# Yoii-Inc/zk-mpc

Hardware: AMD Instinct MI355X
Metric: R1CS constraints/sec (prove), Groth16 BLS12-377 (higher is better)
Workload: dtype u32x13 (29-bit limbs, int64 accumulate); 1 GPU; mul-chain R1CS, n=2^20-2 constraints, QAP domain 2^20, local prove; constraints=1048574, parties=1

## Files before the change

bindings/hip_ffi.rs:

```rust
#![allow(non_camel_case_types, dead_code, clippy::too_many_arguments)]
use std::os::raw::{c_char, c_void};

pub const ZK_OK: i32 = 0;
pub const ZK_ERR_HIP: i32 = -1;
pub const ZK_ERR_ARG: i32 = -2;
pub const ZK_ERR_NOMEM: i32 = -3;
pub const ZK_ERR_STATE: i32 = -4;
pub const ZK_ERR_MAC: i32 = -5;
pub const ZK_OP_MUL: i32 = 0;
pub const ZK_OP_ADD: i32 = 1;
pub const ZK_OP_SUB: i32 = 2;
pub const ZK_OP_NEG: i32 = 3;
pub const ZK_GT_EXPONENT_MULTIPLE: i32 = 3;

#[repr(C)] pub struct ZkCtx { _private: [u8; 0] }
#[repr(C)] pub struct ZkBases { _private: [u8; 0] }
#[repr(C)] pub struct ZkR1cs { _private: [u8; 0] }
#[repr(C)] pub struct ZkPk { _private: [u8; 0] }
#[repr(C)] pub struct ZkRng { _private: [u8; 0] }

#[repr(C)]
#[derive(Clone, Copy)]
pub struct ZkFr {
    pub l: [u64; 4],
// ... 199 lines not shown
    pub fn zk_fr_vec_op_dev(ctx: *mut ZkCtx, op: i32, a_dev: *const c_void, b_dev: *const c_void, out_dev: *mut c_void, n: usize) -> i32;
    pub fn zk_fr_vec_scale_dev(ctx: *mut ZkCtx, a_dev: *const c_void, k_host: *const ZkFr, out_dev: *mut c_void, n: usize) -> i32;
    pub fn zk_fr_batch_product_in_place(ctx: *mut ZkCtx, selfs_host: *mut ZkFr, others_host: *const ZkFr, n: usize) -> i32;
    pub fn zk_fr_ntt_dev(ctx: *mut ZkCtx, buf_dev: *mut c_void, log_n: u32, inverse: i32, coset: i32) -> i32;
    pub fn zk_fr_fft_in_place(ctx: *mut ZkCtx, vec_host: *mut ZkFr, n: usize, log_n: u32, inverse: i32, coset: i32) -> i32;
    pub fn zk_fr_divide_by_vanishing_on_coset_dev(ctx: *mut ZkCtx, evals_dev: *mut c_void, log_n: u32) -> i32;
    pub fn zk_fr_divide_by_vanishing_on_coset_in_place(ctx: *mut ZkCtx, evals_host: *mut ZkFr, log_n: u32) -> i32;
    pub fn zk_msm_g1(ctx: *mut ZkCtx, bases_host: *const ZkG1Affine, n_bases: usize, scalars_host: *const ZkFr, n_scalars: usize, out_host: *mut ZkG1Projective) -> i32;
    pub fn zk_msm_g2(ctx: *mut ZkCtx, bases_host: *const ZkG2Affine, n_bases: usize, scalars_host: *const ZkFr, n_scalars: usize, out_host: *mut ZkG2Projective) -> i32;
    pub fn zk_msm_g1_strided(ctx: *mut ZkCtx, bases_host: *const c_void, n_bases: usize, layout: *const ZkAffineLayout, scalars_host: *const ZkFr, n_scalars: usize, out_host: *mut ZkG1Projective) -> i32;
    pub fn zk_msm_g2_strided(ctx: *mut ZkCtx, bases_host: *const c_void, n_bases: usize, layout: *const ZkAffineLayout, scalars_host: *const ZkFr, n_scalars: usize, out_host: *mut ZkG2Projective) -> i32;
    pub fn zk_bases_cache_config(ctx: *mut ZkCtx, budget_bytes: usize, precompute_after: i32) -> i32;
    pub fn zk_bases_cache_trust(ctx: *mut ZkCtx, fingerprint_only: i32) -> i32;
    pub fn zk_bases_cache_drop(ctx: *mut ZkCtx) -> i32;
    pub fn zk_bases_cache_sync(ctx: *mut ZkCtx) -> i32;
    pub fn zk_bases_cache_stats(ctx: *mut ZkCtx, out: *mut u64 ) -> i32;
    pub fn zk_bases_cache_stats2(ctx: *mut ZkCtx, out: *mut u64 ) -> i32;
    pub fn zk_msm_speculate(ctx: *mut ZkCtx, on: i32) -> i32;
    pub fn zk_msm_speculate_stats(ctx: *mut ZkCtx, out: *mut u64 ) -> i32;
    pub fn zk_bases_upload_g1(ctx: *mut ZkCtx, bases_host: *const ZkG1Affine, n: usize, out: *mut *mut ZkBases) -> i32;
    pub fn zk_bases_upload_g2(ctx: *mut ZkCtx, bases_host: *const ZkG2Affine, n: usize, out: *mut *mut ZkBases) -> i32;
    pub fn zk_bases_free(ctx: *mut ZkCtx, b: *mut ZkBases) -> i32;
    pub fn zk_bases_precompute(ctx: *mut ZkCtx, b: *mut ZkBases) -> i32;
    pub fn zk_bases_precompute_as(ctx: *mut ZkCtx, b: *mut ZkBases, layout: i32) -> i32;
    pub fn zk_bases_precompute_note(b: *const ZkBases) -> *const c_char;
    pub fn zk_bases_window_bits(b: *const ZkBases) -> u32;
    pub fn zk_bases_len(b: *const ZkBases) -> usize;
    pub fn zk_msm_g1_dev(ctx: *mut ZkCtx, bases: *const ZkBases, base_offset: usize, scalars_dev: *const c_void, n: usize, out_host: *mut ZkG1Projective) -> i32;
    pub fn zk_msm_g2_dev(ctx: *mut ZkCtx, bases: *const ZkBases, base_offset: usize, scalars_dev: *const c_void, n: usize, out_host: *mut ZkG2Projective) -> i32;
    pub fn zk_msm_g1_multi_dev(ctx: *mut ZkCtx, bases: *const ZkBases, base_offset: usize, scalars_dev: *const c_void, n: usize, stride: usize, count: usize, outs_host: *mut ZkG1Projective) -> i32;
    pub fn zk_msm_g2_multi_dev(ctx: *mut ZkCtx, bases: *const ZkBases, base_offset: usize, scalars_dev: *const c_void, n: usize, stride: usize, count: usize, outs_host: *mut ZkG2Projective) -> i32;
    pub fn zk_fixed_base_g1_dev(ctx: *mut ZkCtx, gen_k_host: *const ZkFr, scalars_dev: *const c_void, n: usize, out: *mut *mut ZkBases) -> i32;
    pub fn zk_fixed_base_g2_dev(ctx: *mut ZkCtx, gen_k_host: *const ZkFr, scalars_dev: *const c_void, n: usize, out: *mut *mut ZkBases) -> i32;
    pub fn zk_bases_download_g1(ctx: *mut ZkCtx, b: *const ZkBases, offset: usize, n: usize, out_host: *mut ZkG1Affine) -> i32;
    pub fn zk_bases_download_g2(ctx: *mut ZkCtx, b: *const ZkBases, offset: usize, n: usize, out_host: *mut ZkG2Affine) -> i32;
    pub fn zk_point_serialized_size(group: i32, compressed: i32) -> usize;
    pub fn zk_bases_serialize(ctx: *mut ZkCtx, b: *const ZkBases, offset: usize, n: usize, compressed: i32, out_host: *mut u8) -> i32;
    pub fn zk_bases_deserialize_uncompressed(ctx: *mut ZkCtx, group: i32, bytes_host: *const u8, n: usize, out: *mut *mut ZkBases) -> i32;
    pub fn zk_bases_deserialize_compressed(ctx: *mut ZkCtx, group: i32, bytes_host: *const u8, n: usize, out: *mut *mut ZkBases) -> i32;
    pub fn zk_vk_serialized_size(pk: *const ZkPk, compressed: i32) -> usize;
    pub fn zk_pk_serialized_size(pk: *const ZkPk, compressed: i32) -> usize;
    pub fn zk_vk_serialize(ctx: *mut ZkCtx, pk: *const ZkPk, compressed: i32, out_host: *mut u8, cap: usize) -> i32;
    pub fn zk_pk_serialize(ctx: *mut ZkCtx, pk: *const ZkPk, compressed: i32, out_host: *mut u8, cap: usize) -> i32;
    pub fn zk_pk_deserialize(ctx: *mut ZkCtx, bytes_host: *const u8, len: usize, compressed: i32, out: *mut *mut ZkPk) -> i32;
    pub fn zk_kzg_srs_serialized_size(n_powers_g: usize, n_powers_gamma_g: usize, compressed: i32) -> usize;
    pub fn zk_kzg_srs_serialize(ctx: *mut ZkCtx, powers_g: *const ZkBases, powers_gamma_g: *const ZkBases, h: *const ZkG2Affine, beta_h: *const ZkG2Affine, compressed: i32, out_host: *mut u8, cap: usize) -> i32;
    pub fn zk_kzg_srs_deserialize(ctx: *mut ZkCtx, bytes_host: *const u8, len: usize, compressed: i32, powers_g: *mut *mut ZkBases, powers_gamma_g: *mut *mut ZkBases, h: *mut ZkG2Affine, beta_h: *mut ZkG2Affine) -> i32;
    pub fn zk_msm_batch_dev(ctx: *mut ZkCtx, n_jobs: usize, bases: *const *const ZkBases, base_offsets: *const usize, scalars_dev: *const *const c_void, lens: *const usize, outs: *const *mut c_void) -> i32;
    pub fn zk_g1_add(a: *const ZkG1Projective, b: *const ZkG1Projective, out: *mut ZkG1Projective) -> i32;
    pub fn zk_g2_add(a: *const ZkG2Projective, b: *const ZkG2Projective, out: *mut ZkG2Projective) -> i32;
    pub fn zk_g1_neg(a: *const ZkG1Projective, out: *mut ZkG1Projective) -> i32;
    pub fn zk_g2_neg(a: *const ZkG2Projective, out: *mut ZkG2Projective) -> i32;
    pub fn zk_g1_mul(a: *const ZkG1Projective, k: *const ZkFr, out: *mut ZkG1Projective) -> i32;
    pub fn zk_g2_mul(a: *const ZkG2Projective, k: *const ZkFr, out: *mut ZkG2Projective) -> i32;
    pub fn zk_g1_from_affine(a: *const ZkG1Affine, out: *mut ZkG1Projective) -> i32;
    pub fn zk_g2_from_affine(a: *const ZkG2Affine, out: *mut ZkG2Projective) -> i32;
    pub fn zk_g1_serialize(a: *const ZkG1Projective, out: *mut u8 ) -> i32;
    pub fn zk_g2_serialize(a: *const ZkG2Projective, out: *mut u8 ) -> i32;
    pub fn zk_fr_add(a: *const ZkFr, b: *const ZkFr, out: *mut ZkFr) -> i32;
    pub fn zk_fr_sub(a: *const ZkFr, b: *const ZkFr, out: *mut ZkFr) -> i32;
    pub fn zk_fr_mul(a: *const ZkFr, b: *const ZkFr, out: *mut ZkFr) -> i32;
    pub fn zk_fq_add(a: *const ZkFq, b: *const ZkFq, out: *mut ZkFq) -> i32;
    pub fn zk_fq_sub(a: *const ZkFq, b: *const ZkFq, out: *mut ZkFq) -> i32;
    pub fn zk_fq_mul(a: *const ZkFq, b: *const ZkFq, out: *mut ZkFq) -> i32;
    pub fn zk_fq_neg5_almost_raw(a13: *const u32 , out13: *mut u32 ) -> i32;
    pub fn zk_fr_lazy_raw(op: i32, in9s: *const u32, out9s: *mut u32) -> i32;
    pub fn zk_fq_lazy_raw(op: i32, in13s: *const u32, out13s: *mut u32) -> i32;
    pub fn zk_fq_mul2(a: *const ZkFq, b: *const ZkFq, c: *const ZkFq, d: *const ZkFq, out: *mut ZkFq) -> i32;
    pub fn zk_fr_inverse(a: *const ZkFr, out: *mut ZkFr) -> i32;
    pub fn zk_fr_pow(a: *const ZkFr, e: u64, out: *mut ZkFr) -> i32;
    pub fn zk_fr_from_canonical(canon: *const u64 , out: *mut ZkFr) -> i32;
    pub fn zk_fr_to_canonical(a: *const ZkFr, canon: *mut u64 ) -> i32;
    pub fn zk_r1cs_upload(ctx: *mut ZkCtx, m: *const ZkR1csHost, out: *mut *mut ZkR1cs) -> i32;
    pub fn zk_r1cs_free(ctx: *mut ZkCtx, r: *mut ZkR1cs) -> i32;
    pub fn zk_r1cs_mul_chain(ctx: *mut ZkCtx, n: usize, out: *mut *mut ZkR1cs) -> i32;
    pub fn zk_mul_chain_assignment_dev(ctx: *mut ZkCtx, n: usize, w0: *const ZkFr, w1: *const ZkFr, z_dev: *mut c_void) -> i32;
    pub fn zk_pk_upload(ctx: *mut ZkCtx, pk: *const ZkPkHost, out: *mut *mut ZkPk) -> i32;
    pub fn zk_pk_free(ctx: *mut ZkCtx, pk: *mut ZkPk) -> i32;
    pub fn zk_groth16_setup(ctx: *mut ZkCtx, r1cs: *const ZkR1cs, alpha: *const ZkFr, beta: *const ZkFr, gamma: *const ZkFr, delta: *const ZkFr, tau: *const ZkFr, g1_k: *const ZkFr, g2_k: *const ZkFr, out: *mut *mut ZkPk) -> i32;
    pub fn zk_pk_query_len(pk: *const ZkPk, which: i32) -> usize;
    pub fn zk_pk_query_bases(pk: *const ZkPk, which: i32) -> *const ZkBases;
    pub fn zk_msm_mul_levels(ctx: *mut ZkCtx, levels: i32) -> i32;
    pub fn zk_pk_mul_levels(pk: *const ZkPk) -> u32;
    pub fn zk_msm_mul_levels_clamp(window_bits: u32, levels: u32) -> u32;
    pub fn zk_pk_download_g1(ctx: *mut ZkCtx, pk: *const ZkPk, which: i32, offset: usize, n: usize, out: *mut ZkG1Affine) -> i32;
    pub fn zk_pk_download_g2(ctx: *mut ZkCtx, pk: *const ZkPk, which: i32, offset: usize, n: usize, out: *mut ZkG2Affine) -> i32;
    pub fn zk_pk_vk_g1(pk: *const ZkPk, which: i32, out: *mut ZkG1Affine) -> i32;
    pub fn zk_pk_vk_g2(pk: *const ZkPk, which: i32, out: *mut ZkG2Affine) -> i32;
    pub fn zk_groth16_witness_map_dev(ctx: *mut ZkCtx, r1cs: *const ZkR1cs, z_dev: *const c_void, h_dev: *mut c_void) -> i32;
    pub fn zk_r1cs_domain_log(r1cs: *const ZkR1cs) -> u32;
    pub fn zk_groth16_witness_map_pre_dev(ctx: *mut ZkCtx, r1cs: *const ZkR1cs, z_dev: *const c_void, include_instance: i32, a_dev: *mut c_void, b_dev: *mut c_void, c_dev: *mut c_void) -> i32;
    pub fn zk_groth16_witness_map_post_dev(ctx: *mut ZkCtx, r1cs: *const ZkR1cs, ab_dev: *mut c_void, c_dev: *const c_void) -> i32;
    pub fn zk_groth16_hint_next_dev(ctx: *mut ZkCtx, z_next_dev: *const c_void) -> i32;
    pub fn zk_groth16_chain_fronts(ctx: *mut ZkCtx, on: i32) -> i32;
    pub fn zk_groth16_msms_presort_dev(ctx: *mut ZkCtx, pk: *const ZkPk, r1cs: *const ZkR1cs, z_dev: *const c_void) -> i32;
    pub fn zk_groth16_msms_begin_dev(ctx: *mut ZkCtx, pk: *const ZkPk, r: *const ZkR1cs, z: *const c_void) -> i32;
    pub fn zk_groth16_msms_dev(ctx: *mut ZkCtx, pk: *const ZkPk, r1cs: *const ZkR1cs, z_dev: *const c_void, h_dev: *const c_void, out_g1: *mut ZkG1Projective , out_g2: *mut ZkG2Projective) -> i32;
    pub fn zk_groth16_prove_dev(ctx: *mut ZkCtx, pk: *const ZkPk, r1cs: *const ZkR1cs, z_dev: *const c_void, r: *const ZkFr, s: *const ZkFr, proof_out: *mut u8 ) -> i32;
    pub fn zk_groth16_prove_batch_dev(ctx: *mut ZkCtx, pk: *const ZkPk, r1cs: *const ZkR1cs, count: usize, z_dev: *const c_void, r: *const ZkFr, s: *const ZkFr, proofs_out: *mut u8) -> i32;
    pub fn zk_groth16_prove_batch(ctx: *mut ZkCtx, pk: *const ZkPk, r1cs: *const ZkR1cs, count: usize, z_host: *const ZkFr, r: *const ZkFr, s: *const ZkFr, proofs_out: *mut u8) -> i32;
    pub fn zk_groth16_prove_multi(ctxs: *const *mut ZkCtx, pks: *const *const ZkPk, r1css: *const *const ZkR1cs, n_ctx: i32, z_dev0: *const c_void, r: *const ZkFr, s: *const ZkFr, proof_out: *mut u8 ) -> i32;
    pub fn zk_groth16_multi_plan(pk: *const ZkPk, r1cs: *const ZkR1cs, n_ctx: i32, out: *mut c_char, cap: usize, written: *mut usize) -> i32;
    pub fn zk_groth16_prove(ctx: *mut ZkCtx, pk: *const ZkPk, r1cs: *const ZkR1cs, z_host: *const ZkFr, r: *const ZkFr, s: *const ZkFr, proof_out: *mut u8 ) -> i32;
    pub fn zk_groth16_prove_queued(ctx: *mut ZkCtx, pk: *const ZkPk, r1cs: *const ZkR1cs, z_host: *const ZkFr, r: *const ZkFr, s: *const ZkFr, z_next_host: *const ZkFr, proof_out: *mut u8 ) -> i32;
    pub fn zk_gt_exponent_multiple() -> i32;
    pub fn zk_pairing_products(ctx: *mut ZkCtx, p: *const ZkG1Affine, q: *const ZkG2Affine, pairs: usize, count: usize, outs: *mut ZkGt) -> i32;
    pub fn zk_pairing_products_host(p: *const ZkG1Affine, q: *const ZkG2Affine, pairs: usize, count: usize, outs: *mut ZkGt) -> i32;
    pub fn zk_gt_is_one(a: *const ZkGt) -> i32;
    pub fn zk_gt_eq(a: *const ZkGt, b: *const ZkGt) -> i32;
    pub fn zk_gt_mul(a: *const ZkGt, b: *const ZkGt, out: *mut ZkGt) -> i32;
    pub fn zk_groth16_verify_batch(ctx: *mut ZkCtx, pk: *const ZkPk, count: usize, inputs_host: *const ZkFr, inputs_per_proof: usize, proofs_host: *const u8, ok: *mut i32) -> i32;
    pub fn zk_groth16_verify_host(vk: *const ZkVkHost, inputs: *const ZkFr, n_inputs: usize, proof: *const u8 , ok: *mut i32) -> i32;
    pub fn zk_marlin_verify_host(vk: *const ZkMarlinVkHost, inputs: *const ZkFr, n_inputs: usize, proof: *const u8, proof_len: usize, ok: *mut i32) -> i32;
    pub fn zk_marlin_verify_batch(ctx: *mut ZkCtx, vk: *const ZkMarlinVkHost, count: usize, inputs_host: *const ZkFr, inputs_per_proof: usize, proofs_host: *const u8, offsets: *const usize, ok: *mut i32) -> i32;
    pub fn zk_fr_powers_dev(ctx: *mut ZkCtx, base: *const ZkFr, start: *const ZkFr, n: usize, out_dev: *mut c_void) -> i32;
    pub fn zk_fr_batch_inverse_dev(ctx: *mut ZkCtx, v_dev: *mut c_void, n: usize) -> i32;
    pub fn zk_poly_evaluate_dev(ctx: *mut ZkCtx, coeffs_dev: *const c_void, n: usize, point: *const ZkFr, out: *mut ZkFr) -> i32;
    pub fn zk_poly_evaluate_batch_dev(ctx: *mut ZkCtx, polys: *const ZkPolyRef, points: *const ZkFr, count: usize, out: *mut ZkFr) -> i32;
    pub fn zk_poly_divide_by_linear_dev(ctx: *mut ZkCtx, coeffs_dev: *const c_void, n: usize, z: *const ZkFr, q_dev: *mut c_void, rem: *mut ZkFr) -> i32;
    pub fn zk_poly_divide_by_vanishing_dev(ctx: *mut ZkCtx, coeffs_dev: *const c_void, n: usize, log_domain: u32, q_dev: *mut c_void, r_dev: *mut c_void) -> i32;
    pub fn zk_poly_mul_dev(ctx: *mut ZkCtx, a_dev: *const c_void, na: usize, b_dev: *const c_void, nb: usize, out_dev: *mut c_void) -> i32;
    pub fn zk_kzg_commit_dev(ctx: *mut ZkCtx, powers_g: *const ZkBases, coeffs_dev: *const c_void, n: usize, powers_gamma_g: *const ZkBases, blind_dev: *const c_void, n_blind: usize, out: *mut ZkG1Projective) -> i32;
    pub fn zk_kzg_open_dev(ctx: *mut ZkCtx, powers_g: *const ZkBases, coeffs_dev: *const c_void, n: usize, point: *const ZkFr, powers_gamma_g: *const ZkBases, blind_dev: *const c_void, n_blind: usize, w_out: *mut ZkG1Projective, random_v_out: *mut ZkFr) -> i32;
    pub fn zk_r1cs_matvec_dev(ctx: *mut ZkCtx, r1cs: *const ZkR1cs, which: i32, z_dev: *const c_void, out_dev: *mut c_void, out_len: usize) -> i32;
    pub fn zk_fr_gather_dev(ctx: *mut ZkCtx, src_dev: *const c_void, idx_dev: *const u32, n: usize, out_dev: *mut c_void) -> i32;
    pub fn zk_marlin_round3_f_evals_dev(ctx: *mut ZkCtx, on_k: *const ZkMarlinMatrixEvals , k_size: usize, alpha: *const ZkFr, beta: *const ZkFr, eta: *const ZkFr , vh_alpha_vh_beta: *const ZkFr, f_out_dev: *mut c_void) -> i32;
    pub fn zk_marlin_round3_ab_evals_dev(ctx: *mut ZkCtx, on_b: *const ZkMarlinMatrixEvals , b_size: usize, alpha: *const ZkFr, beta: *const ZkFr, eta: *const ZkFr , vh_alpha_vh_beta: *const ZkFr, a_out_dev: *mut c_void, b_out_dev: *mut c_void) -> i32;
    pub fn zk_marlin_proof_max_size() -> usize;
    pub fn zk_marlin_prove(ctx: *mut ZkCtx, index: *const ZkMarlinIndex, powers_g: *const ZkBases, powers_gamma_g: *const ZkBases, z_dev: *const c_void, zk_rng: *mut ZkRng, mask_on_device: i32, proof_out: *mut u8, cap: usize, proof_len: *mut usize) -> i32;
    pub fn zk_she_vec_op_dev(ctx: *mut ZkCtx, op: i32, a_dev: *const c_void, b_dev: *const c_void, out_dev: *mut c_void, n: usize) -> i32;
    pub fn zk_she_vec_scale_dev(ctx: *mut ZkCtx, a_dev: *const c_void, k: *const ZkFq753, out_dev: *mut c_void, n: usize) -> i32;
    pub fn zk_she_negacyclic_mul_dev(ctx: *mut ZkCtx, a_dev: *const c_void, b_dev: *const c_void, out_dev: *mut c_void, n: usize, batch: usize) -> i32;
    pub fn zk_she_ciphertext_mul_dev(ctx: *mut ZkCtx, x_dev: *const c_void, y_dev: *const c_void, out_dev: *mut c_void, n: usize, batch: usize) -> i32;
    pub fn zk_she_encrypt_dev(ctx: *mut ZkCtx, e_dev: *const c_void, pk_a_dev: *const c_void, pk_b_dev: *const c_void, r_dev: *const c_void, p: *const ZkFq753, out_dev: *mut c_void, n: usize, batch: usize) -> i32;
    pub fn zk_she_decrypt_dev(ctx: *mut ZkCtx, ct_dev: *const c_void, sk_dev: *const c_void, out_dev: *mut c_void, n: usize, batch: usize) -> i32;
    pub fn zk_she_encode_dev(ctx: *mut ZkCtx, plain_fr_dev: *const c_void, out_dev: *mut c_void, n: usize, batch: usize) -> i32;
    pub fn zk_she_decode_dev(ctx: *mut ZkCtx, enc_dev: *const c_void, out_fr_dev: *mut c_void, n: usize, batch: usize) -> i32;
    pub fn zk_comm_unique_id(out: *mut u8 ) -> i32;
    pub fn zk_comm_init(ctx: *mut ZkCtx, id: *const u8 , rank: i32, n_parties: i32) -> i32;
    pub fn zk_comm_destroy(ctx: *mut ZkCtx) -> i32;
    pub fn zk_comm_info(ctx: *mut ZkCtx, n_ranks: *mut i32, rank: *mut i32, device: *mut i32, rccl_version: *mut i32, lib_path: *mut c_char, lib_path_cap: usize) -> i32;
    pub fn zk_comm_set_open_pattern(ctx: *mut ZkCtx, pattern: i32) -> i32;
    pub fn zk_open_sum_fr_dev(ctx: *mut ZkCtx, v_dev: *const c_void, n: usize, out_dev: *mut c_void) -> i32;
    pub fn zk_groth16_prove_shared(ctx: *mut ZkCtx, pk: *const ZkPk, r1cs: *const ZkR1cs, z_share_dev: *const c_void, r_share: *const ZkFr, s_share: *const ZkFr, tx_dev: *const c_void, ty_dev: *const c_void, tz_dev: *const c_void, net: *const ZkNetVtable, proof: *mut u8 , bytes_sent: *mut u64) -> i32;
    pub fn zk_groth16_prove_shared_spdz(ctx: *mut ZkCtx, pk: *const ZkPk, r1cs: *const ZkR1cs, z_lanes_dev: *const *const c_void , r_lanes: *const ZkFr , s_lanes: *const ZkFr , tx_lanes_dev: *const *const c_void , ty_lanes_dev: *const *const c_void , tz_lanes_dev: *const *const c_void , net: *const ZkNetVtable, proof: *mut u8 , bytes_sent: *mut u64) -> i32;
    pub fn zk_marlin_prove_shared(ctx: *mut ZkCtx, index: *const ZkMarlinIndex, powers_g: *const ZkBases, powers_gamma_g: *const ZkBases, z_share_dev: *const c_void, zk_rng: *mut ZkRng, mask_on_device: i32, tx: *const c_void, ty: *const c_void, tz: *const c_void, net: *const ZkNetVtable, proof_out: *mut u8, cap: usize, proof_len: *mut usize, bytes_sent: *mut u64) -> i32;
    pub fn zk_marlin_prove_shared_spdz(ctx: *mut ZkCtx, index: *const ZkMarlinIndex, powers_g: *const ZkBases, powers_gamma_g: *const ZkBases, z_lanes_dev: *const *const c_void , zk_rng: *mut ZkRng, mask_on_device: i32, tx_lanes: *const *const c_void , ty_lanes: *const *const c_void , tz_lanes: *const *const c_void , net: *const ZkNetVtable, proof_out: *mut u8, cap: usize, proof_len: *mut usize, bytes_sent: *mut u64) -> i32;
    pub fn zk_mpc_fft_in_place(ctx: *mut ZkCtx, vec_host: *mut c_void, n: usize, layout: *const ZkMpcFieldLayout, log_n: u32, inverse: i32, coset: i32) -> i32;
    pub fn zk_mpc_divide_by_vanishing_on_coset_in_place(ctx: *mut ZkCtx, evals_host: *mut c_void, layout: *const ZkMpcFieldLayout, log_n: u32) -> i32;
    pub fn zk_mpc_batch_product_in_place(ctx: *mut ZkCtx, selfs_host: *mut c_void, others_host: *const c_void, n: usize, layout: *const ZkMpcFieldLayout, triple_host: *const *const ZkFr, net: *const ZkNetVtable, bytes_sent: *mut u64) -> i32;
    pub fn zk_mpc_msm_g1(ctx: *mut ZkCtx, bases_host: *const c_void, n_bases: usize, base_layout: *const ZkMpcGroupLayout, scalars_host: *const c_void, n_scalars: usize, scalar_layout: *const ZkMpcFieldLayout, out_lanes: *mut ZkG1Projective , scalars_public: *mut i32) -> i32;
    pub fn zk_mpc_msm_g2(ctx: *mut ZkCtx, bases_host: *const c_void, n_bases: usize, base_layout: *const ZkMpcGroupLayout, scalars_host: *const c_void, n_scalars: usize, scalar_layout: *const ZkMpcFieldLayout, out_lanes: *mut ZkG2Projective , scalars_public: *mut i32) -> i32;
    pub fn zk_fr_sum_parties_dev(ctx: *mut ZkCtx, gathered_dev: *const c_void, n_parties: usize, n: usize, out_dev: *mut c_void) -> i32;
    pub fn zk_beaver_combine_dev(ctx: *mut ZkCtx, sx_open_dev: *const c_void, oy_open_dev: *const c_void, tx_dev: *const c_void, ty_dev: *const c_void, tz_dev: *const c_void, out_dev: *mut c_void, n: usize) -> i32;
    pub fn zk_fr_vec_is_zero_dev(ctx: *mut ZkCtx, v_dev: *const c_void, n: usize, is_zero: *mut i32) -> i32;
    pub fn zk_fr_random_dev(ctx: *mut ZkCtx, key32: *const u8, stream_id: u64, out_dev: *mut c_void, n: usize) -> i32;
    pub fn zk_fsrng_new(seed_bytes: *const u8, len: usize, out: *mut *mut ZkRng) -> i32;
    pub fn zk_fsrng_absorb(rng: *mut ZkRng, bytes: *const u8, len: usize) -> i32;
    pub fn zk_rng_from_seed(seed: *const u8 , rounds: i32, out: *mut *mut ZkRng) -> i32;
    pub fn zk_rng_free(rng: *mut ZkRng) -> i32;
    pub fn zk_rng_next_u64(rng: *mut ZkRng, out: *mut u64) -> i32;
    pub fn zk_rng_next_u128(rng: *mut ZkRng, out: *mut u64 ) -> i32;
    pub fn zk_rng_next_fr(rng: *mut ZkRng, out: *mut ZkFr) -> i32;
    pub fn zk_rng_fill_fr(rng: *mut ZkRng, out: *mut ZkFr, n: usize) -> i32;
    pub fn zk_rng_fill_bytes(rng: *mut ZkRng, out: *mut u8, n: usize) -> i32;
    pub fn zk_blake2s(data: *const u8, len: usize, out: *mut u8 ) -> i32;
// ... 17 lines not shown
```

include/zkmpc_hip.h:

```cpp
#ifndef ZKMPC_HIP_H
#define ZKMPC_HIP_H

#include <stddef.h>
#include <stdint.h>

#ifdef __cplusplus
extern "C" {
#endif

#define ZK_OK 0
#define ZK_ERR_HIP -1
#define ZK_ERR_ARG -2
#define ZK_ERR_NOMEM -3
#define ZK_ERR_STATE -4
#define ZK_ERR_MAC -5

typedef struct zk_ctx zk_ctx;
typedef struct zk_bases zk_bases;
typedef struct zk_r1cs zk_r1cs;
typedef struct zk_pk zk_pk;
typedef struct zk_rng zk_rng;

typedef struct { uint64_t l[4]; } zk_fr;
typedef struct { uint64_t l[6]; } zk_fq;
// ... 63 lines not shown
                  size_t n, zk_g2_projective* out_host);
int zk_msm_g1_multi_dev(zk_ctx* ctx, const zk_bases* bases, size_t base_offset, const void* scalars_dev,
                        size_t n, size_t stride, size_t count, zk_g1_projective* outs_host);
int zk_msm_g2_multi_dev(zk_ctx* ctx, const zk_bases* bases, size_t base_offset, const void* scalars_dev,
                        size_t n, size_t stride, size_t count, zk_g2_projective* outs_host);
int zk_fixed_base_g1_dev(zk_ctx* ctx, const zk_fr* gen_k_host, const void* scalars_dev, size_t n, zk_bases** out);
int zk_fixed_base_g2_dev(zk_ctx* ctx, const zk_fr* gen_k_host, const void* scalars_dev, size_t n, zk_bases** out);
int zk_bases_download_g1(zk_ctx* ctx, const zk_bases* b, size_t offset, size_t n, zk_g1_affine* out_host);
int zk_bases_download_g2(zk_ctx* ctx, const zk_bases* b, size_t offset, size_t n, zk_g2_affine* out_host);

size_t zk_point_serialized_size(int group, int compressed);
int zk_bases_serialize(zk_ctx* ctx, const zk_bases* b, size_t offset, size_t n, int compressed, uint8_t* out_host);
int zk_bases_deserialize_uncompressed(zk_ctx* ctx, int group, const uint8_t* bytes_host, size_t n, zk_bases** out);
int zk_bases_deserialize_compressed(zk_ctx* ctx, int group, const uint8_t* bytes_host, size_t n, zk_bases** out);

size_t zk_vk_serialized_size(const zk_pk* pk, int compressed);
size_t zk_pk_serialized_size(const zk_pk* pk, int compressed);
int zk_vk_serialize(zk_ctx* ctx, const zk_pk* pk, int compressed, uint8_t* out_host, size_t cap);
int zk_pk_serialize(zk_ctx* ctx, const zk_pk* pk, int compressed, uint8_t* out_host, size_t cap);
int zk_pk_deserialize(zk_ctx* ctx, const uint8_t* bytes_host, size_t len, int compressed, zk_pk** out);
size_t zk_kzg_srs_serialized_size(size_t n_powers_g, size_t n_powers_gamma_g, int compressed);
int zk_kzg_srs_serialize(zk_ctx* ctx, const zk_bases* powers_g, const zk_bases* powers_gamma_g, const zk_g2_affine* h,
                         const zk_g2_affine* beta_h, int compressed, uint8_t* out_host, size_t cap);
int zk_kzg_srs_deserialize(zk_ctx* ctx, const uint8_t* bytes_host, size_t len, int compressed, zk_bases** powers_g,
                           zk_bases** powers_gamma_g, zk_g2_affine* h, zk_g2_affine* beta_h);

int zk_msm_batch_dev(zk_ctx* ctx, size_t n_jobs, const zk_bases* const* bases, const size_t* base_offsets,
                     const void* const* scalars_dev, const size_t* lens, void* const* outs);

int zk_g1_add(const zk_g1_projective* a, const zk_g1_projective* b, zk_g1_projective* out);
int zk_g2_add(const zk_g2_projective* a, const zk_g2_projective* b, zk_g2_projective* out);
int zk_g1_neg(const zk_g1_projective* a, zk_g1_projective* out);
int zk_g2_neg(const zk_g2_projective* a, zk_g2_projective* out);
int zk_g1_mul(const zk_g1_projective* a, const zk_fr* k, zk_g1_projective* out);
int zk_g2_mul(const zk_g2_projective* a, const zk_fr* k, zk_g2_projective* out);
int zk_g1_from_affine(const zk_g1_affine* a, zk_g1_projective* out);
int zk_g2_from_affine(const zk_g2_affine* a, zk_g2_projective* out);
int zk_g1_serialize(const zk_g1_projective* a, uint8_t out[48]);
int zk_g2_serialize(const zk_g2_projective* a, uint8_t out[96]);
int zk_fr_add(const zk_fr* a, const zk_fr* b, zk_fr* out);
int zk_fr_sub(const zk_fr* a, const zk_fr* b, zk_fr* out);
int zk_fr_mul(const zk_fr* a, const zk_fr* b, zk_fr* out);
int zk_fq_add(const zk_fq* a, const zk_fq* b, zk_fq* out);
int zk_fq_sub(const zk_fq* a, const zk_fq* b, zk_fq* out);
int zk_fq_mul(const zk_fq* a, const zk_fq* b, zk_fq* out);
int zk_fq_neg5_almost_raw(const uint32_t a13[13], uint32_t out13[13]);
int zk_fr_lazy_raw(int op, const uint32_t* in9s, uint32_t* out9s);
int zk_fq_lazy_raw(int op, const uint32_t* in13s, uint32_t* out13s);
int zk_fq_mul2(const zk_fq* a, const zk_fq* b, const zk_fq* c, const zk_fq* d, zk_fq* out);
int zk_fr_inverse(const zk_fr* a, zk_fr* out);
int zk_fr_pow(const zk_fr* a, uint64_t e, zk_fr* out);
int zk_fr_from_canonical(const uint64_t canon[4], zk_fr* out);
int zk_fr_to_canonical(const zk_fr* a, uint64_t canon[4]);

typedef struct {
    size_t num_constraints, num_instance, num_witness;
    const uint32_t* a_row_ptr; const uint32_t* a_col; const zk_fr* a_coeff;
    const uint32_t* b_row_ptr; const uint32_t* b_col; const zk_fr* b_coeff;
    const uint32_t* c_row_ptr; const uint32_t* c_col; const zk_fr* c_coeff;
} zk_r1cs_host;
int zk_r1cs_upload(zk_ctx* ctx, const zk_r1cs_host* m, zk_r1cs** out);
int zk_r1cs_free(zk_ctx* ctx, zk_r1cs* r);
int zk_r1cs_mul_chain(zk_ctx* ctx, size_t n, zk_r1cs** out);
int zk_mul_chain_assignment_dev(zk_ctx* ctx, size_t n, const zk_fr* w0, const zk_fr* w1, void* z_dev);

typedef struct {
    zk_g1_affine alpha_g1, beta_g1, delta_g1;
    zk_g2_affine beta_g2, delta_g2;
    const zk_g1_affine* a_query;    size_t a_len;
    const zk_g1_affine* b_g1_query; size_t b_g1_len;
    const zk_g2_affine* b_g2_query; size_t b_g2_len;
    const zk_g1_affine* h_query;    size_t h_len;
    const zk_g1_affine* l_query;    size_t l_len;
} zk_pk_host;
int zk_pk_upload(zk_ctx* ctx, const zk_pk_host* pk, zk_pk** out);
int zk_pk_free(zk_ctx* ctx, zk_pk* pk);
int zk_groth16_setup(zk_ctx* ctx, const zk_r1cs* r1cs, const zk_fr* alpha, const zk_fr* beta,
                     const zk_fr* gamma, const zk_fr* delta, const zk_fr* tau,
                     const zk_fr* g1_k, const zk_fr* g2_k, zk_pk** out);
size_t zk_pk_query_len(const zk_pk* pk, int which);
const zk_bases* zk_pk_query_bases(const zk_pk* pk, int which);
int zk_msm_mul_levels(zk_ctx* ctx, int levels);
uint32_t zk_pk_mul_levels(const zk_pk* pk);
uint32_t zk_msm_mul_levels_clamp(uint32_t window_bits, uint32_t levels);
int zk_pk_download_g1(zk_ctx* ctx, const zk_pk* pk, int which, size_t offset, size_t n, zk_g1_affine* out);
int zk_pk_download_g2(zk_ctx* ctx, const zk_pk* pk, int which, size_t offset, size_t n, zk_g2_affine* out);
int zk_pk_vk_g1(const zk_pk* pk, int which, zk_g1_affine* out);
int zk_pk_vk_g2(const zk_pk* pk, int which, zk_g2_affine* out);

int zk_groth16_witness_map_dev(zk_ctx* ctx, const zk_r1cs* r1cs, const void* z_dev, void* h_dev);
uint32_t zk_r1cs_domain_log(const zk_r1cs* r1cs);
int zk_groth16_witness_map_pre_dev(zk_ctx* ctx, const zk_r1cs* r1cs, const void* z_dev,
                                   int include_instance, void* a_dev, void* b_dev, void* c_dev);
int zk_groth16_witness_map_post_dev(zk_ctx* ctx, const zk_r1cs* r1cs, void* ab_dev, const void* c_dev);
int zk_groth16_hint_next_dev(zk_ctx* ctx, const void* z_next_dev);
int zk_groth16_chain_fronts(zk_ctx* ctx, int on);
int zk_groth16_msms_presort_dev(zk_ctx* ctx, const zk_pk* pk, const zk_r1cs* r1cs, const void* z_dev);
int zk_groth16_msms_begin_dev(zk_ctx* ctx, const zk_pk* pk, const zk_r1cs* r, const void* z);
int zk_groth16_msms_dev(zk_ctx* ctx, const zk_pk* pk, const zk_r1cs* r1cs, const void* z_dev,
                        const void* h_dev, zk_g1_projective out_g1[4], zk_g2_projective* out_g2);
int zk_groth16_prove_dev(zk_ctx* ctx, const zk_pk* pk, const zk_r1cs* r1cs, const void* z_dev,
                         const zk_fr* r, const zk_fr* s, uint8_t proof_out[192]);
int zk_groth16_prove_batch_dev(zk_ctx* ctx, const zk_pk* pk, const zk_r1cs* r1cs, size_t count, const void* z_dev,
                               const zk_fr* r, const zk_fr* s, uint8_t* proofs_out);
int zk_groth16_prove_batch(zk_ctx* ctx, const zk_pk* pk, const zk_r1cs* r1cs, size_t count, const zk_fr* z_host,
                           const zk_fr* r, const zk_fr* s, uint8_t* proofs_out);
int zk_groth16_prove_multi(zk_ctx* const* ctxs, const zk_pk* const* pks, const zk_r1cs* const* r1css, int n_ctx, const void* z_dev0,
                           const zk_fr* r, const zk_fr* s, uint8_t proof_out[192]);
int zk_groth16_multi_plan(const zk_pk* pk, const zk_r1cs* r1cs, int n_ctx, char* out, size_t cap, size_t* written);
int zk_groth16_prove(zk_ctx* ctx, const zk_pk* pk, const zk_r1cs* r1cs, const zk_fr* z_host,
                     const zk_fr* r, const zk_fr* s, uint8_t proof_out[192]);
int zk_groth16_prove_queued(zk_ctx* ctx, const zk_pk* pk, const zk_r1cs* r1cs, const zk_fr* z_host,
                            const zk_fr* r, const zk_fr* s, const zk_fr* z_next_host, uint8_t proof_out[192]);

#define ZK_GT_EXPONENT_MULTIPLE 3
int zk_gt_exponent_multiple(void);
typedef struct { zk_fq c[12]; } zk_gt;
int zk_pairing_products(zk_ctx* ctx, const zk_g1_affine* p, const zk_g2_affine* q, size_t pairs, size_t count, zk_gt* outs);
int zk_pairing_products_host(const zk_g1_affine* p, const zk_g2_affine* q, size_t pairs, size_t count, zk_gt* outs);
int zk_gt_is_one(const zk_gt* a);
int zk_gt_eq(const zk_gt* a, const zk_gt* b);
int zk_gt_mul(const zk_gt* a, const zk_gt* b, zk_gt* out);
int zk_groth16_verify_batch(zk_ctx* ctx, const zk_pk* pk, size_t count, const zk_fr* inputs_host, size_t inputs_per_proof,
                            const uint8_t* proofs_host, int* ok);
typedef struct {
    zk_g1_affine alpha_g1;
    zk_g2_affine beta_g2, gamma_g2, delta_g2;
    const zk_g1_affine* gamma_abc_g1; size_t gamma_abc_len;
} zk_vk_host;
int zk_groth16_verify_host(const zk_vk_host* vk, const zk_fr* inputs, size_t n_inputs, const uint8_t proof[192], int* ok);

typedef struct {
    const uint8_t* ivk_bytes; size_t ivk_len;
    zk_g1_affine g, gamma_g;
    zk_g2_affine h, beta_h;
    zk_g1_affine shift_h, shift_k;
} zk_marlin_vk_host;
int zk_marlin_verify_host(const zk_marlin_vk_host* vk, const zk_fr* inputs, size_t n_inputs, const uint8_t* proof, size_t proof_len, int* ok);
int zk_marlin_verify_batch(zk_ctx* ctx, const zk_marlin_vk_host* vk, size_t count, const zk_fr* inputs_host, size_t inputs_per_proof,
                           const uint8_t* proofs_host, const size_t* offsets, int* ok);

int zk_fr_powers_dev(zk_ctx* ctx, const zk_fr* base, const zk_fr* start, size_t n, void* out_dev);
int zk_fr_batch_inverse_dev(zk_ctx* ctx, void* v_dev, size_t n);
int zk_poly_evaluate_dev(zk_ctx* ctx, const void* coeffs_dev, size_t n, const zk_fr* point, zk_fr* out);
typedef struct { const void* ptr; size_t n; } zk_poly_ref;
int zk_poly_evaluate_batch_dev(zk_ctx* ctx, const zk_poly_ref* polys, const zk_fr* points, size_t count, zk_fr* out);
int zk_poly_divide_by_linear_dev(zk_ctx* ctx, const void* coeffs_dev, size_t n, const zk_fr* z, void* q_dev, zk_fr* rem);
int zk_poly_divide_by_vanishing_dev(zk_ctx* ctx, const void* coeffs_dev, size_t n, uint32_t log_domain, void* q_dev, void* r_dev);
int zk_poly_mul_dev(zk_ctx* ctx, const void* a_dev, size_t na, const void* b_dev, size_t nb, void* out_dev);
int zk_kzg_commit_dev(zk_ctx* ctx, const zk_bases* powers_g, const void* coeffs_dev, size_t n,
                      const zk_bases* powers_gamma_g, const void* blind_dev, size_t n_blind, zk_g1_projective* out);
int zk_kzg_open_dev(zk_ctx* ctx, const zk_bases* powers_g, const void* coeffs_dev, size_t n, const zk_fr* point,
                    const zk_bases* powers_gamma_g, const void* blind_dev, size_t n_blind,
                    zk_g1_projective* w_out, zk_fr* random_v_out);

int zk_r1cs_matvec_dev(zk_ctx* ctx, const zk_r1cs* r1cs, int which, const void* z_dev, void* out_dev, size_t out_len);
int zk_fr_gather_dev(zk_ctx* ctx, const void* src_dev, const uint32_t* idx_dev, size_t n, void* out_dev);
typedef struct { const void* row; const void* col; const void* val; const void* row_col; } zk_marlin_matrix_evals;
int zk_marlin_round3_f_evals_dev(zk_ctx* ctx, const zk_marlin_matrix_evals on_k[3], size_t k_size, const zk_fr* alpha,
                                 const zk_fr* beta, const zk_fr eta[3], const zk_fr* vh_alpha_vh_beta, void* f_out_dev);
int zk_marlin_round3_ab_evals_dev(zk_ctx* ctx, const zk_marlin_matrix_evals on_b[3], size_t b_size, const zk_fr* alpha,
                                  const zk_fr* beta, const zk_fr eta[3], const zk_fr* vh_alpha_vh_beta, void* a_out_dev,
                                  void* b_out_dev);

typedef struct {
    size_t num_constraints, num_variables, num_non_zero, num_instance;
// ... 112 lines not shown
```

zk-mpc_amd/_lib.py:

```python
from __future__ import annotations

import ctypes as C
import os

_HERE = os.path.dirname(os.path.abspath(__file__))
LIB_PATH = os.path.join(_HERE, "lib", "libzkmpc_hip.so")

ZK_OK = 0
OP_MUL, OP_ADD, OP_SUB, OP_NEG = 0, 1, 2, 3


class ZkError(RuntimeError):
    pass


class Fr(C.Structure):
    _fields_ = [("l", C.c_uint64 * 4)]


class Fq(C.Structure):
    _fields_ = [("l", C.c_uint64 * 6)]


class MarlinMatrixEvals(C.Structure):
# ... 74 lines not shown
    "zk_ctx_sync": (_I, [_P]),
    "zk_ctx_stream": (_P, [_P]),
    "zk_version": (_I, []),
    "zk_groth16_prove_shared": (_I, [_P, _P, _P, _P, _P, _P, _P, _P, _P, _P, _P, _P]),
    "zk_groth16_prove_shared_spdz": (_I, [_P, _P, _P, _P, _P, _P, _P, _P, _P, _P, _P, _P]),
    "zk_selftest_exception_barrier": (_I, [_I]),
    "zk_dev_alloc": (_I, [_P, _SZ, C.POINTER(_P)]),
    "zk_dev_free": (_I, [_P, _P]),
    "zk_memcpy_h2d": (_I, [_P, _P, _P, _SZ]),
    "zk_memcpy_d2h": (_I, [_P, _P, _P, _SZ]),
    "zk_fr_vec_op_dev": (_I, [_P, _I, _P, _P, _P, _SZ]),
    "zk_fr_vec_scale_dev": (_I, [_P, _P, _P, _P, _SZ]),
    "zk_fr_batch_product_in_place": (_I, [_P, _P, _P, _SZ]),
    "zk_fr_ntt_dev": (_I, [_P, _P, _U32, _I, _I]),
    "zk_fr_fft_in_place": (_I, [_P, _P, _SZ, _U32, _I, _I]),
    "zk_fr_divide_by_vanishing_on_coset_dev": (_I, [_P, _P, _U32]),
    "zk_msm_g1": (_I, [_P, _P, _SZ, _P, _SZ, _P]),
    "zk_msm_g2": (_I, [_P, _P, _SZ, _P, _SZ, _P]),
    "zk_msm_g1_strided": (_I, [_P, _P, _SZ, _P, _P, _SZ, _P]),
    "zk_msm_g2_strided": (_I, [_P, _P, _SZ, _P, _P, _SZ, _P]),
    "zk_bases_cache_config": (_I, [_P, _SZ, _I]),
    "zk_bases_cache_trust": (_I, [_P, _I]),
    "zk_msm_speculate": (_I, [_P, _I]),
    "zk_msm_speculate_stats": (_I, [_P, _P]),
    "zk_bases_cache_drop": (_I, [_P]),
    "zk_bases_cache_sync": (_I, [_P]),
    "zk_bases_cache_stats": (_I, [_P, _P]),
    "zk_bases_cache_stats2": (_I, [_P, _P]),
    "zk_mpc_fft_in_place": (_I, [_P, _P, _SZ, _P, _U32, _I, _I]),
    "zk_mpc_divide_by_vanishing_on_coset_in_place": (_I, [_P, _P, _P, _U32]),
    "zk_mpc_batch_product_in_place": (_I, [_P, _P, _P, _SZ, _P, _P, _P, _P]),
    "zk_mpc_msm_g1": (_I, [_P, _P, _SZ, _P, _P, _SZ, _P, _P, _P]),
    "zk_mpc_msm_g2": (_I, [_P, _P, _SZ, _P, _P, _SZ, _P, _P, _P]),
    "zk_fr_divide_by_vanishing_on_coset_in_place": (_I, [_P, _P, _U32]),
    "zk_bases_upload_g1": (_I, [_P, _P, _SZ, C.POINTER(_P)]),
    "zk_bases_upload_g2": (_I, [_P, _P, _SZ, C.POINTER(_P)]),
    "zk_bases_free": (_I, [_P, _P]),
    "zk_bases_precompute": (_I, [_P, _P]),
    "zk_bases_precompute_as": (_I, [_P, _P, _I]),
    "zk_bases_precompute_note": (C.c_char_p, [_P]),
    "zk_bases_len": (_SZ, [_P]),
    "zk_bases_window_bits": (_U32, [_P]),
    "zk_msm_g1_dev": (_I, [_P, _P, _SZ, _P, _SZ, _P]),
    "zk_msm_g2_dev": (_I, [_P, _P, _SZ, _P, _SZ, _P]),
    "zk_msm_g1_multi_dev": (_I, [_P, _P, _SZ, _P, _SZ, _SZ, _SZ, _P]),
    "zk_msm_g2_multi_dev": (_I, [_P, _P, _SZ, _P, _SZ, _SZ, _SZ, _P]),
    "zk_fixed_base_g1_dev": (_I, [_P, _P, _P, _SZ, C.POINTER(_P)]),
    "zk_fixed_base_g2_dev": (_I, [_P, _P, _P, _SZ, C.POINTER(_P)]),
    "zk_bases_download_g1": (_I, [_P, _P, _SZ, _SZ, _P]),
    "zk_bases_download_g2": (_I, [_P, _P, _SZ, _SZ, _P]),
    "zk_g1_add": (_I, [_P, _P, _P]),
    "zk_g2_add": (_I, [_P, _P, _P]),
    "zk_g1_neg": (_I, [_P, _P]),
    "zk_g2_neg": (_I, [_P, _P]),
    "zk_g1_mul": (_I, [_P, _P, _P]),
    "zk_g2_mul": (_I, [_P, _P, _P]),
    "zk_g1_from_affine": (_I, [_P, _P]),
    "zk_g2_from_affine": (_I, [_P, _P]),
    "zk_g1_serialize": (_I, [_P, _P]),
    "zk_g2_serialize": (_I, [_P, _P]),
    "zk_fr_add": (_I, [_P, _P, _P]),
    "zk_fr_sub": (_I, [_P, _P, _P]),
    "zk_fr_mul": (_I, [_P, _P, _P]),
    "zk_fq_add": (_I, [_P, _P, _P]),
    "zk_fq_sub": (_I, [_P, _P, _P]),
    "zk_fq_mul": (_I, [_P, _P, _P]),
    "zk_fq_mul2": (_I, [_P, _P, _P, _P, _P]),
    "zk_fq_neg5_almost_raw": (_I, [_P, _P]),
    "zk_fq_lazy_raw": (_I, [_I, _P, _P]),
    "zk_fr_lazy_raw": (_I, [_I, _P, _P]),
    "zk_fr_from_canonical": (_I, [_P, _P]),
    "zk_fr_to_canonical": (_I, [_P, _P]),
    "zk_r1cs_upload": (_I, [_P, _P, C.POINTER(_P)]),
    "zk_r1cs_free": (_I, [_P, _P]),
    "zk_r1cs_mul_chain": (_I, [_P, _SZ, C.POINTER(_P)]),
    "zk_mul_chain_assignment_dev": (_I, [_P, _SZ, _P, _P, _P]),
    "zk_pk_upload": (_I, [_P, _P, C.POINTER(_P)]),
    "zk_pk_free": (_I, [_P, _P]),
    "zk_groth16_setup": (_I, [_P, _P, _P, _P, _P, _P, _P, _P, _P, C.POINTER(_P)]),
    "zk_pk_query_len": (_SZ, [_P, _I]),
    "zk_pk_query_bases": (_P, [_P, _I]),
    "zk_msm_mul_levels": (_I, [_P, _I]),
    "zk_pk_mul_levels": (_U32, [_P]),
    "zk_msm_mul_levels_clamp": (_U32, [_U32, _U32]),
    "zk_pk_download_g1": (_I, [_P, _P, _I, _SZ, _SZ, _P]),
    "zk_pk_download_g2": (_I, [_P, _P, _I, _SZ, _SZ, _P]),
    "zk_pk_vk_g1": (_I, [_P, _I, _P]),
    "zk_pk_vk_g2": (_I, [_P, _I, _P]),
    "zk_groth16_witness_map_dev": (_I, [_P, _P, _P, _P]),
    "zk_r1cs_domain_log": (_U32, [_P]),
    "zk_groth16_witness_map_pre_dev": (_I, [_P, _P, _P, _I, _P, _P, _P]),
    "zk_groth16_witness_map_post_dev": (_I, [_P, _P, _P, _P]),
    "zk_groth16_msms_dev": (_I, [_P, _P, _P, _P, _P, _P, _P]),
    "zk_groth16_msms_presort_dev": (_I, [_P, _P, _P, _P]),
    "zk_groth16_msms_begin_dev": (_I, [_P, _P, _P, _P]),
    "zk_groth16_hint_next_dev": (_I, [_P, _P]),
    "zk_groth16_chain_fronts": (_I, [_P, _I]),
    "zk_groth16_prove_dev": (_I, [_P, _P, _P, _P, _P, _P, _P]),
    "zk_groth16_prove_batch_dev": (_I, [_P, _P, _P, _SZ, _P, _P, _P, _P]),
    "zk_groth16_prove_batch": (_I, [_P, _P, _P, _SZ, _P, _P, _P, _P]),
    "zk_groth16_prove_multi": (_I, [_P, _P, _P, _I, _P, _P, _P, _P]),
    "zk_groth16_multi_plan": (_I, [_P, _P, _I, C.c_char_p, _SZ, C.POINTER(_SZ)]),
    "zk_groth16_prove": (_I, [_P, _P, _P, _P, _P, _P, _P]),
    "zk_groth16_prove_queued": (_I, [_P, _P, _P, _P, _P, _P, _P, _P]),
    "zk_host_alloc": (_I, [_P, _SZ, C.POINTER(_P)]),
    "zk_host_free": (_I, [_P, _P]),
    "zk_fr_powers_dev": (_I, [_P, _P, _P, _SZ, _P]),
    "zk_fr_batch_inverse_dev": (_I, [_P, _P, _SZ]),
    "zk_poly_evaluate_dev": (_I, [_P, _P, _SZ, _P, _P]),
    "zk_poly_evaluate_batch_dev": (_I, [_P, _P, _P, _SZ, _P]),
    "zk_poly_divide_by_linear_dev": (_I, [_P, _P, _SZ, _P, _P, _P]),
    "zk_poly_divide_by_vanishing_dev": (_I, [_P, _P, _SZ, _U32, _P, _P]),
    "zk_poly_mul_dev": (_I, [_P, _P, _SZ, _P, _SZ, _P]),
    "zk_kzg_commit_dev": (_I, [_P, _P, _P, _SZ, _P, _P, _SZ, _P]),
    "zk_kzg_open_dev": (_I, [_P, _P, _P, _SZ, _P, _P, _P, _SZ, _P, _P]),
    "zk_point_serialized_size": (_SZ, [_I, _I]),
    "zk_bases_serialize": (_I, [_P, _P, _SZ, _SZ, _I, _P]),
    "zk_bases_deserialize_uncompressed": (_I, [_P, _I, _P, _SZ, C.POINTER(_P)]),
    "zk_bases_deserialize_compressed": (_I, [_P, _I, _P, _SZ, C.POINTER(_P)]),
    "zk_msm_batch_dev": (_I, [_P, _SZ, _P, _P, _P, _P, _P]),
    "zk_vk_serialized_size": (_SZ, [_P, _I]),
    "zk_pk_serialized_size": (_SZ, [_P, _I]),
    "zk_vk_serialize": (_I, [_P, _P, _I, _P, _SZ]),
    "zk_pk_serialize": (_I, [_P, _P, _I, _P, _SZ]),
    "zk_pk_deserialize": (_I, [_P, _P, _SZ, _I, C.POINTER(_P)]),
    "zk_kzg_srs_serialized_size": (_SZ, [_SZ, _SZ, _I]),
    "zk_kzg_srs_serialize": (_I, [_P, _P, _P, _P, _P, _I, _P, _SZ]),
    "zk_kzg_srs_deserialize": (_I, [_P, _P, _SZ, _I, C.POINTER(_P), C.POINTER(_P), _P, _P]),
    "zk_comm_unique_id": (_I, [_P]),
    "zk_comm_init": (_I, [_P, _P, _I, _I]),
    "zk_comm_destroy": (_I, [_P]),
    "zk_comm_info": (_I, [_P, C.POINTER(_I), C.POINTER(_I), C.POINTER(_I), C.POINTER(_I), C.c_char_p, _SZ]),
    "zk_comm_set_open_pattern": (_I, [_P, _I]),
    "zk_open_sum_fr_dev": (_I, [_P, _P, _SZ, _P]),
    "zk_memcpy_d2d": (_I, [_P, _P, _P, _SZ]),
    "zk_dev_zero": (_I, [_P, _P, _SZ]),
    "zk_fr_inverse": (_I, [_P, _P]),
    "zk_fr_pow": (_I, [_P, C.c_uint64, _P]),
    "zk_r1cs_matvec_dev": (_I, [_P, _P, _I, _P, _P, _SZ]),
    "zk_fr_gather_dev": (_I, [_P, _P, _P, _SZ, _P]),
    "zk_marlin_round3_f_evals_dev": (_I, [_P, _P, _SZ, _P, _P, _P, _P, _P]),
    "zk_marlin_round3_ab_evals_dev": (_I, [_P, _P, _SZ, _P, _P, _P, _P, _P, _P]),
    "zk_marlin_proof_max_size": (_SZ, []),
    "zk_marlin_prove": (_I, [_P, _P, _P, _P, _P, _P, _I, _P, _SZ, _P]),
    "zk_marlin_prove_shared": (_I, [_P, _P, _P, _P, _P, _P, _I, _P, _P, _P, _P, _P, _SZ, _P, _P]),
    "zk_marlin_prove_shared_spdz": (_I, [_P, _P, _P, _P, _P, _P, _I, _P, _P, _P, _P, _P, _SZ, _P, _P]),
    "zk_she_vec_op_dev": (_I, [_P, _I, _P, _P, _P, _SZ]),
    "zk_she_vec_scale_dev": (_I, [_P, _P, _P, _P, _SZ]),
    "zk_she_negacyclic_mul_dev": (_I, [_P, _P, _P, _P, _SZ, _SZ]),
    "zk_she_ciphertext_mul_dev": (_I, [_P, _P, _P, _P, _SZ, _SZ]),
    "zk_she_encrypt_dev": (_I, [_P, _P, _P, _P, _P, _P, _P, _SZ, _SZ]),
    "zk_she_decrypt_dev": (_I, [_P, _P, _P, _P, _SZ, _SZ]),
    "zk_she_encode_dev": (_I, [_P, _P, _P, _SZ, _SZ]),
    "zk_she_decode_dev": (_I, [_P, _P, _P, _SZ, _SZ]),
    "zk_fr_sum_parties_dev": (_I, [_P, _P, _SZ, _SZ, _P]),
    "zk_beaver_combine_dev": (_I, [_P, _P, _P, _P, _P, _P, _P, _SZ]),
    "zk_fr_vec_is_zero_dev": (_I, [_P, _P, _SZ, _P]),
    "zk_fr_random_dev": (_I, [_P, _P, C.c_uint64, _P, _SZ]),
    "zk_fsrng_new": (_I, [_P, _SZ, C.POINTER(_P)]),
    "zk_fsrng_absorb": (_I, [_P, _P, _SZ]),
    "zk_rng_from_seed": (_I, [_P, _I, C.POINTER(_P)]),
    "zk_rng_free": (_I, [_P]),
    "zk_rng_next_u64": (_I, [_P, _P]),
    "zk_rng_next_u128": (_I, [_P, _P]),
    "zk_rng_next_fr": (_I, [_P, _P]),
    "zk_rng_fill_fr": (_I, [_P, _P, _SZ]),
# ... 47 lines not shown
```

zk-mpc_amd/api.py:

```python
from __future__ import annotations

import ctypes as C

import numpy as np

from . import _lib
from ._lib import ZkError


def _ptr(a: np.ndarray):
    return a.ctypes.data_as(C.c_void_p)


def _fr_struct(limbs4) -> _lib.Fr:
    f = _lib.Fr()
    for i in range(4):
        f.l[i] = int(limbs4[i])
    return f


class HostBuf:

    def __init__(self, ctx: "Context", nbytes: int):
        self.ctx, self.nbytes = ctx, nbytes
# ... 768 lines not shown
        return out

    def groth16_verify_batch(self, pk: "ProvingKey", inputs_mont: np.ndarray, proofs) -> np.ndarray:
        data = b"".join(proofs) if isinstance(proofs, (list, tuple)) else bytes(proofs)
        if len(data) % 192:
            raise ValueError("proofs must be a whole number of 192-byte proofs")
        count = len(data) // 192
        inp = np.ascontiguousarray(inputs_mont, dtype=np.uint64).reshape(count, -1, 4) if count else np.zeros((0, 0, 4), np.uint64)
        buf = np.frombuffer(data, dtype=np.uint8)
        ok = np.zeros(count, dtype=np.int32)
        self._ck(self.lib.zk_groth16_verify_batch(self.h, pk.h, count, _ptr(inp), inp.shape[1], _ptr(buf), _ptr(ok)))
        return ok

    def groth16_verify(self, pk: "ProvingKey", inputs_mont: np.ndarray, proof: bytes) -> bool:
        return bool(self.groth16_verify_batch(pk, np.asarray(inputs_mont, dtype=np.uint64).reshape(1, -1, 4), proof)[0])

    def diag_fq12(self, op: int, a: np.ndarray, b: np.ndarray) -> np.ndarray:
        cases = np.ascontiguousarray(np.stack([a, b], axis=1), dtype=np.uint64)
        out = np.zeros((cases.shape[0], 72), dtype=np.uint64)
        self._ck(self.lib.zk_diag_fq12_dev(self.h, op, _ptr(cases), _ptr(out), cases.shape[0]))
        return out


class Bases:
    def __init__(self, ctx: Context, h, group: int, owned: bool = True):
        self.ctx, self.h, self.group, self.owned = ctx, h, group, owned

    def __len__(self):
        return self.ctx.lib.zk_bases_len(self.h)

    def precompute(self, layout: int = 0):
        if layout:
            self.ctx._ck(self.ctx.lib.zk_bases_precompute_as(self.ctx.h, self.h, layout))
        else:
            self.ctx._ck(self.ctx.lib.zk_bases_precompute(self.ctx.h, self.h))

    def precompute_note(self) -> str:
        return (self.ctx.lib.zk_bases_precompute_note(self.h) or b"").decode()

    def download(self, offset: int = 0, n: int = None) -> np.ndarray:
        n = len(self) - offset if n is None else n
        out = np.zeros((n, 12 if self.group == 1 else 24), dtype=np.uint64)
        fn = self.ctx.lib.zk_bases_download_g1 if self.group == 1 else self.ctx.lib.zk_bases_download_g2
        self.ctx._ck(fn(self.ctx.h, self.h, offset, n, _ptr(out)))
        return out

    def serialize(self, compressed: bool = True, offset: int = 0, n: int = None) -> bytes:
        n = len(self) - offset if n is None else n
        per = self.ctx.lib.zk_point_serialized_size(self.group, int(compressed))
        out = np.zeros(max(n * per, 1), dtype=np.uint8)
        self.ctx._ck(self.ctx.lib.zk_bases_serialize(self.ctx.h, self.h, offset, n, int(compressed), _ptr(out)))
        return out[: n * per].tobytes()

    def free(self):
        if self.h and self.owned:
            self.ctx.lib.zk_bases_free(self.ctx.h, self.h)
        self.h = None


class R1cs:
    def __init__(self, ctx: Context, h, nc: int, ni: int, nw: int):
        self.ctx, self.h = ctx, h
        self.num_constraints, self.num_instance, self.num_witness = nc, ni, nw

    @property
    def domain_log(self) -> int:
        return self.ctx.lib.zk_r1cs_domain_log(self.h)

    def free(self):
        if self.h:
            self.ctx.lib.zk_r1cs_free(self.ctx.h, self.h)
            self.h = None


class ProvingKey:
    QUERIES = {"a_query": 0, "b_g1_query": 1, "b_g2_query": 2, "h_query": 3, "l_query": 4, "gamma_abc_g1": 5}

    def __init__(self, ctx: Context, h):
        self.ctx, self.h = ctx, h

    def mul_levels(self) -> int:
        return self.ctx.lib.zk_pk_mul_levels(self.h)

    def query_len(self, name: str) -> int:
        return self.ctx.lib.zk_pk_query_len(self.h, self.QUERIES[name])

    def download(self, name: str, offset: int = 0, n: int = None) -> np.ndarray:
        which = self.QUERIES[name]
        n = self.query_len(name) - offset if n is None else n
        if which == 2:
            out = np.zeros((n, 24), dtype=np.uint64)
            self.ctx._ck(self.ctx.lib.zk_pk_download_g2(self.ctx.h, self.h, which, offset, n, _ptr(out)))
        else:
            out = np.zeros((n, 12), dtype=np.uint64)
            self.ctx._ck(self.ctx.lib.zk_pk_download_g1(self.ctx.h, self.h, which, offset, n, _ptr(out)))
        return out

    def query_bases(self, name: str) -> "Bases":
        which = self.QUERIES[name]
        h = self.ctx.lib.zk_pk_query_bases(self.h, which)
        return Bases(self.ctx, C.c_void_p(h), 2 if which == 2 else 1, owned=False)

    def vk_g1(self, which: int) -> np.ndarray:
        out = np.zeros(12, dtype=np.uint64)
        self.ctx._ck(self.ctx.lib.zk_pk_vk_g1(self.h, which, _ptr(out)))
        return out

    def vk_g2(self, which: int) -> np.ndarray:
        out = np.zeros(24, dtype=np.uint64)
        self.ctx._ck(self.ctx.lib.zk_pk_vk_g2(self.h, which, _ptr(out)))
        return out

    def verify_host(self, inputs_mont, proof: bytes) -> bool:
        return groth16_verify_host(self.vk_g1(0), self.vk_g2(0), self.vk_g2(2), self.vk_g2(1), self.download("gamma_abc_g1"), inputs_mont, proof)

    def free(self):
        if self.h:
            self.ctx.lib.zk_pk_free(self.ctx.h, self.h)
            self.h = None


def _pairing_args(p, q, pairs):
    p = np.ascontiguousarray(p, dtype=np.uint64).reshape(-1, 12)
    q = np.ascontiguousarray(q, dtype=np.uint64).reshape(-1, 24)
    if pairs < 1 or p.shape[0] != q.shape[0] or p.shape[0] == 0 or p.shape[0] % pairs:
        raise ValueError("pairing_products: need as many G1 as G2 points, a positive multiple of `pairs`")
    return p, q, p.shape[0] // pairs


def _ck_host(rc: int, what: str):
    if rc != _lib.ZK_OK:
        raise ZkError("%s failed (%d)" % (what, rc))


def gt_exponent_multiple() -> int:
    return _lib.load().zk_gt_exponent_multiple()


def pairing_products_host(p: np.ndarray, q: np.ndarray, pairs: int = 1) -> np.ndarray:
    p, q, count = _pairing_args(p, q, pairs)
    out = np.zeros((count, 72), dtype=np.uint64)
    _ck_host(_lib.load().zk_pairing_products_host(_ptr(p), _ptr(q), pairs, count, _ptr(out)), "zk_pairing_products_host")
    return out


def gt_is_one(a: np.ndarray) -> bool:
    return bool(_lib.load().zk_gt_is_one(_ptr(np.ascontiguousarray(a, dtype=np.uint64))))


def gt_eq(a: np.ndarray, b: np.ndarray) -> bool:
    return bool(_lib.load().zk_gt_eq(_ptr(np.ascontiguousarray(a, dtype=np.uint64)), _ptr(np.ascontiguousarray(b, dtype=np.uint64))))


def gt_mul(a: np.ndarray, b: np.ndarray) -> np.ndarray:
    out = np.zeros(72, dtype=np.uint64)
    _ck_host(_lib.load().zk_gt_mul(_ptr(np.ascontiguousarray(a, dtype=np.uint64)), _ptr(np.ascontiguousarray(b, dtype=np.uint64)), _ptr(out)), "zk_gt_mul")
    return out


def gt_to_w_basis(gt: np.ndarray) -> list:
    from . import convert as cv
    row = np.asarray(gt, dtype=np.uint64).reshape(72)
    out = [0] * 12
    for i in range(2):
        for j in range(3):
            for h in range(2):
# ... 39 lines not shown
```

zk-mpc_amd/csrc/fixed_base.hip:

```cpp
#include "../../include/zkmpc_hip.h"
#include "devutil.cuh"
#include "internal.hpp"

using namespace zk;

namespace {

constexpr int FB_WINDOWS = 32;
constexpr int NORM_CHUNK = 16;

template <class F>
struct AffArg { uint32_t w[2 * F::WORDS]; };

template <class F>
__global__ void __launch_bounds__(64) k_fb_table(uint32_t* table, AffArg<F> gen) {
    uint32_t t = blockIdx.x * blockDim.x + threadIdx.x;
    if (t >= FB_WINDOWS * 256) return;
    uint32_t j = t >> 8, d = t & 255;
    Affine<F> g = aff_load<F>(gen.w);
    uint32_t k[8] = {0, 0, 0, 0, 0, 0, 0, 0};
    k[j >> 2] = d << (8 * (j & 3));
    XYZZ<F> r = xyzz_scalar_mul<F>(g, k, (int)(j >> 2) + 1);
    aff_store16<F>(table, t, xyzz_to_affine<F>(r));
}
// ... 223 lines not shown
            if (e == hipSuccess) e = hipStreamSynchronize(ctx->stream);
            if (e != hipSuccess) { fail_free(wide); ZK_HIP(ctx, e); }
            (void)hipFree(b->pre);
            b->pre = wide;
            b->pre_stride = (uint32_t)words;
            b->pre_note = form == 3 ? "limbs, both signs (256 B per point)" : "one point per 128-byte line";
        }
    } else if (layout > 1) {
        fail_free(nullptr);
        ZK_FAIL(ctx, ZK_ERR_ARG, "zk_bases_precompute_as: layouts 2 and 3 are G1 forms");
    }
    return ZK_OK;
}

}

extern "C" int zk_fixed_base_g1_dev(zk_ctx* ctx, const zk_fr* gen_k, const void* scalars, size_t n, zk_bases** out) {
    ZK_API_BEGIN(ctx)
    return fixed_base_run<G1Field>(ctx, g1_generator(), gen_k, scalars, n, 1, out);
    ZK_API_END
}
extern "C" int zk_fixed_base_g2_dev(zk_ctx* ctx, const zk_fr* gen_k, const void* scalars, size_t n, zk_bases** out) {
    ZK_API_BEGIN(ctx)
    return fixed_base_run<G2Field>(ctx, g2_generator(), gen_k, scalars, n, 2, out);
    ZK_API_END
}

static uint32_t precompute_window_bits(size_t n) {
    uint32_t lg = 0;
    while (((size_t)3 << lg) <= 2 * n) lg++;
    int c0 = lg >= 19 ? 20 : lg >= 16 ? 17 : (lg >= 13 ? std::min((int)lg + 1, 15) : (int)lg + 2);
    if (lg == 16 && n < 65000) c0 = 15;
    const int lo = lg >= 16 ? 13 : 9, hi = lg >= 16 ? 20 : 16;
    if (c0 < lo) c0 = lo;
    if (c0 > hi) c0 = hi;
    const int need = std::min(10, std::max(3, (int)lg - 3));
    const int tries[9] = {0, -1, 1, -2, 2, -3, 3, 4, 5};
    for (int t : tries) {
        int c = c0 + t;
        if (c < lo - 1 || c > 20) continue;
        int W = (255 + c - 1) / c;
        if (255 - c * (W - 1) >= need) return (uint32_t)c;
    }
    return 16;
}

static int precompute_enabled_by_default() {
    const char* e = getenv("ZK_PRECOMP");
    return !e || atoi(e) != 0;
}
int zk_bases_precompute_auto(zk_ctx* ctx, zk_bases* b) {
    return (precompute_enabled_by_default() && b && b->n >= ZK_PRECOMP_MIN_POINTS) ? zk_bases_precompute(ctx, b) : ZK_OK;
}

extern "C" uint32_t zk_bases_window_bits(const zk_bases* b) { return b ? b->c_pre : 0; }
uint32_t zk_precompute_windows(size_t n) { const uint32_t c = precompute_window_bits(n); return (255 + c - 1) / c; }

static int precompute_run(zk_ctx* ctx, zk_bases* b, int layout, uint32_t levels = 0) {
    if (!ctx || layout < 0 || layout > 3) return ZK_ERR_ARG;
    if (!b || b->pre || b->n < ZK_PRECOMP_MIN_POINTS) return ZK_OK;
    const uint32_t c = precompute_window_bits(b->n);
    const uint32_t W = (255 + c - 1) / c;
    levels = zk_msm_mul_levels_clamp(c, levels);
    if (b->group == 1) return precompute_t<G1Field>(ctx, b, c, W, layout, levels);
    return precompute_t<G2Field>(ctx, b, c, W, layout, levels);
}

extern "C" uint32_t zk_msm_mul_levels_clamp(uint32_t c, uint32_t levels) {
    uint32_t M = levels < ZK_MSM_MAX_LEVELS ? levels : ZK_MSM_MAX_LEVELS;
    while (M && c < 2 + M + ZK_MSM_MIN_LOG_NB) M--;
    return M;
}
constexpr uint32_t MUL_LEVELS_DEFAULT = 3;
uint32_t zk_mul_levels_for_key(zk_ctx* ctx, size_t n) {
    if (n < ZK_PRECOMP_MIN_POINTS || !precompute_enabled_by_default()) return 0;
    const uint32_t c = precompute_window_bits(n), W = (255 + c - 1) / c;
    const char* e = getenv("ZK_MSM_MUL_LEVELS");
    const int forced = ctx->mul_levels >= 0 ? ctx->mul_levels : (e && *e ? atoi(e) : -1);
    if (forced >= 0) return zk_msm_mul_levels_clamp(c, (uint32_t)forced);
    uint32_t M = zk_msm_mul_levels_clamp(c, c >= 20 ? MUL_LEVELS_DEFAULT : 0u);
    if (!M) return 0;
    size_t mem_free = 0, mem_total = 0;
    if (hipMemGetInfo(&mem_free, &mem_total) != hipSuccess) { (void)hipGetLastError(); return 0; }
    while (M && (size_t)(M + 1) * W * n * (4 * 256 + 96 + 192) > mem_free / 3) M--;
    return M;
}
int zk_bases_precompute_levels(zk_ctx* ctx, zk_bases* b, uint32_t levels) {
    if (!precompute_enabled_by_default() || !b || b->n < ZK_PRECOMP_MIN_POINTS) return ZK_OK;
    for (uint32_t lv = levels;; lv--) {
        ZK_TRY(precompute_run(ctx, b, 0, lv));
        if (b->pre || lv == 0) return ZK_OK;
    }
}

extern "C" int zk_bases_precompute(zk_ctx* ctx, zk_bases* b) {
    ZK_API_BEGIN(ctx)
    return precompute_run(ctx, b, 0);
    ZK_API_END
}

extern "C" int zk_bases_precompute_as(zk_ctx* ctx, zk_bases* b, int layout) {
    ZK_API_BEGIN(ctx)
    return precompute_run(ctx, b, layout);
    ZK_API_END
}

namespace {
constexpr size_t PRE_SLICE = (size_t)1 << 18;
constexpr size_t PRE_REPACK_SLICE = (size_t)1 << 21;

template <class F>
int precompute_begin_t(zk_ctx* ctx, zk_bases* b, uint32_t c, uint32_t W, size_t budget, ZkPrecompJob** out) {
    const size_t n = b->n, PW = 2 * F::WORDS;
    const size_t packed_bytes = (size_t)W * n * PW * 4, xy_bytes = n * 4 * F::WORDS * 4, scr_bytes = n * F::WORDS * 4;
    if (packed_bytes + xy_bytes + scr_bytes > budget) {
        char msg[256];
        snprintf(msg, sizeof msg, "window multiples skipped for a %zu-point G%d table (c = %u, W = %u: %.2f GB packed): more than the cache's budget", n, b->group, c, W, packed_bytes / 1e9);
        b->pre_note = msg;
        return ZK_OK;
    }
    std::unique_ptr<ZkPrecompJob> j(new ZkPrecompJob());
    j->b = b; j->c = c; j->W = W;
    j->budget = budget;
    (void)ctx;
    *out = j.release();
    return ZK_OK;
}

template <class F>
hipError_t precompute_step_t(ZkPrecompJob* j, hipStream_t st, bool* more) {
    const zk_bases* b = j->b;
    const size_t n = b->n, PW = 2 * F::WORDS;
    *more = true;
    if (j->phase == -1) {
        const size_t packed_bytes = (size_t)j->W * n * PW * 4, xy_bytes = n * 4 * F::WORDS * 4, scr_bytes = n * F::WORDS * 4;
        if (packed_bytes + xy_bytes + scr_bytes > ((size_t)256 << 20)) {
            size_t mem_free = 0, mem_total = 0;
            if (hipMemGetInfo(&mem_free, &mem_total) != hipSuccess) { (void)hipGetLastError(); return hipErrorOutOfMemory; }
            j->budget = std::min(j->budget, mem_free / 3);
        }
        if (packed_bytes + xy_bytes + scr_bytes > j->budget) return hipErrorOutOfMemory;
        if (hipMalloc((void**)&j->packed, packed_bytes) != hipSuccess || hipMalloc((void**)&j->xy, xy_bytes) != hipSuccess ||
            hipMalloc((void**)&j->scr, scr_bytes) != hipSuccess) {
            (void)hipGetLastError();
            return hipErrorOutOfMemory;
        }
        if constexpr (F::WORDS == 12) {
            for (uint32_t words : {64u, 32u}) {
                const size_t bytes = (size_t)j->W * n * words * 4;
                if (packed_bytes + xy_bytes + scr_bytes + bytes > j->budget) continue;
                if (hipMalloc((void**)&j->wide, bytes) != hipSuccess) { j->wide = nullptr; (void)hipGetLastError(); continue; }
                j->wide_words = words;
                break;
            }
        }
        j->phase = 0;
        return hipSuccess;
    }
    if (j->phase == 0) {
        j->phase = j->W > 1 ? 1 : 2;
        j->w = 1; j->pos = 0;
        return hipMemcpyAsync(j->packed, b->dev, n * PW * 4, hipMemcpyDeviceToDevice, st);
    }
    if (j->phase == 1) {
        const size_t lo = j->pos, len = std::min(PRE_SLICE, n - lo), chunks = (len + NORM_CHUNK - 1) / NORM_CHUNK;
        hipLaunchKernelGGL(k_dbl_c<F>, zk_grid(len, 256), 256, 0, st, j->packed + ((size_t)(j->w - 1) * n + lo) * PW, j->xy + lo * 4 * F::WORDS, len, j->c);
        hipLaunchKernelGGL(k_batch_affine<F>, (unsigned)((chunks + 63) / 64), 64, 0, st, j->xy + lo * 4 * F::WORDS, j->packed + ((size_t)j->w * n + lo) * PW,
                           j->scr + lo * F::WORDS, len);
// ... 69 lines not shown
```

zk-mpc_amd/csrc/groth16_batch.hip:

```cpp
#include "../../include/zkmpc_hip.h"
#include "groth16_int.hpp"
#include <algorithm>

using namespace zk;

namespace {

constexpr size_t TAIL_TASKS = 16, PRE_TASKS = 8;

template <class Fn>
void over_ranges(zk_ctx* ctx, size_t count, size_t tasks, const Fn& f) {
    const size_t nt = std::min(count, tasks), per = (count + nt - 1) / nt;
    std::vector<ZkTask<void>> ts;
    for (size_t t = 1; t < nt; t++) {
        const size_t lo = t * per, hi = std::min(count, lo + per);
        if (lo < hi) ts.push_back(zk_async(ctx, [&f, lo, hi] { f(lo, hi); }));
    }
    f(0, std::min(count, per));
    for (auto& t : ts) t.get();
}

int prove_chunk(zk_ctx* ctx, const zk_pk* pk, const zk_r1cs* r, size_t cnt, const char* z, const char* h, const std::function<int()>& front,
                const std::function<void()>& pre_ready, ZkTail* tails, uint8_t* proofs) {
    const ZkG16Jobs T(pk, r, z, h);
    hipStream_t s_sort = ctx->aux[0], s_acc = ctx->acc_stream;
    struct Event {
        hipEvent_t e = nullptr;
        ~Event() { if (e) (void)hipEventDestroy(e); }
    } e0;
    ZK_HIP(ctx, hipEventCreateWithFlags(&e0.e, hipEventDisableTiming));
    ZK_HIP(ctx, hipEventRecord(e0.e, ctx->stream));
    ZK_HIP(ctx, hipStreamWaitEvent(s_sort, e0.e, 0));
    ZkMsmJob J[5];
    struct Streams {
        zk_ctx* ctx;
        ~Streams() {
            (void)hipStreamSynchronize(ctx->aux[0]);
            (void)hipStreamSynchronize(ctx->acc_stream);
            (void)hipStreamSynchronize(ctx->stream);
        }
    } drain{ctx};
    ZkMsmJob* const zj[4] = {&J[0], &J[1], &J[2], &J[3]};
    ZK_TRY(T.sort_z(ctx, zj, s_sort, ZK_SLOT_G16_BATCH, cnt));
    if (!T.l_shared) ZK_TRY(zk_msm_enqueue_sort(ctx, &J[3], s_sort, nullptr));
    ZK_TRY(front());
    ZK_TRY(T.prepare(ctx, 4, &J[4], ZK_SLOT_G16_BATCH, cnt));
    ZK_TRY(zk_msm_enqueue_sort(ctx, &J[4], ctx->stream, nullptr));
    ZK_TRY(zk_msm_enqueue_accum(ctx, &J[0], s_acc));
    ZK_TRY(zk_msm_enqueue_reduce(ctx, &J[0], s_acc));
    for (int j = 1; j <= 3; j++) {
        ZK_TRY(zk_msm_enqueue_accum(ctx, &J[j], s_sort));
        ZK_TRY(zk_msm_enqueue_reduce(ctx, &J[j], s_sort));
    }
    ZK_TRY(zk_msm_enqueue_accum(ctx, &J[4], ctx->stream));
    ZK_TRY(zk_msm_enqueue_reduce(ctx, &J[4], ctx->stream));
    std::vector<zk_g1_projective> a(cnt), b1(cnt), l(cnt), hs(cnt);
    std::vector<zk_g2_projective> b2(cnt);
    ZK_TRY(zk_msm_finish_multi(ctx, &J[0], b2.data()));
    ZK_TRY(zk_msm_finish_multi(ctx, &J[1], a.data()));
    ZK_TRY(zk_msm_finish_multi(ctx, &J[2], b1.data()));
    ZK_TRY(zk_msm_finish_multi(ctx, &J[3], l.data()));
    ZK_TRY(zk_msm_finish_multi(ctx, &J[4], hs.data()));
    pre_ready();
    over_ranges(ctx, cnt, TAIL_TASKS, [&](size_t lo, size_t hi) {
        for (size_t k = lo; k < hi; k++) {
            zk_tail_chain_a(pk, &tails[k], a[k]);
            zk_tail_chain_b(pk, &tails[k], b1[k]);
            zk_tail_chain_2(pk, &tails[k], b2[k]);
            zk_tail_finish(tails[k], hs[k], l[k], proofs + k * 192);
        }
    });
    return ZK_OK;
}

size_t chunk_bytes(const zk_pk* pk, const zk_r1cs* r, size_t cnt) {
    size_t bytes = 0;
    for (const ZkG16Jobs::Job& j : ZkG16Jobs(pk, r, nullptr, nullptr).j) {
        const size_t W = j.tab->pre ? (255 + j.tab->c_pre - 1) / j.tab->c_pre : 32;
        const size_t XW = j.tab->group == 1 ? 48 : 96;
        const size_t buckets = j.tab->pre ? ((size_t)1 << (j.tab->c_pre - 1)) : W * std::max<size_t>(j.n, 16);
        bytes += cnt * (j.n * W * 16 + buckets * XW * 4 * 2);
    }
    return bytes;
}

int batch_plan(zk_ctx* ctx, const zk_pk* pk, const zk_r1cs* r, size_t count, size_t* chunk_out) {
    ZK_TRY(zk_groth16_key_matches(ctx, pk, r));
    const size_t m = r->ni + r->nw, D = (size_t)1 << r->log_d;
    size_t chunk = count;
    for (const ZkG16Jobs::Job& j : ZkG16Jobs(pk, r, nullptr, nullptr).j) chunk = std::min(chunk, zk_msm_multi_chunk(j.tab, j.n));
    size_t free_b = 0, total_b = 0;
    ZK_HIP(ctx, hipMemGetInfo(&free_b, &total_b));
    const double need = (double)count * (double)(m + 6 * D) * 32.0 + (double)chunk_bytes(pk, r, chunk);
    if (need > (double)(free_b / 10 * 9))
        ZK_FAIL(ctx, ZK_ERR_NOMEM, "groth16 batch: the working set of " + std::to_string(count) + " proofs (" +
                                       std::to_string((unsigned long long)(need / 1048576.0)) + " MiB) does not fit the free device memory (" +
                                       std::to_string(free_b >> 20) + " MiB)");
    *chunk_out = chunk;
    return ZK_OK;
}

struct CallMem {
    zk_ctx* ctx;
    void* p = nullptr;
    ~CallMem() {
        if (!p) return;
        (void)hipStreamSynchronize(ctx->stream);
        (void)hipFree(p);
    }
};

int run_batch(zk_ctx* ctx, const zk_pk* pk, const zk_r1cs* r, size_t count, size_t chunk, const void* z_dev, const zk_fr* r_,
              const zk_fr* s_, uint8_t* proofs_out) {
    const size_t m = r->ni + r->nw, D = (size_t)1 << r->log_d;
    ZK_TRY(zk_next_z_drop(ctx, true));
    if (count == 1) return zk_groth16_prove_dev(ctx, pk, r, z_dev, r_, s_, proofs_out);
    ZK_TRY(zk_prover_streams(ctx, 1));
    CallMem wm{ctx};
    ZK_HIP(ctx, hipMalloc(&wm.p, count * 6 * D * 32));
    std::vector<ZkTail> tails(count);
    ZkTask<void> pre_task = zk_async(ctx, [&] {
        over_ranges(ctx, count, PRE_TASKS, [&](size_t lo, size_t hi) {
            for (size_t k = lo; k < hi; k++) {
                zk_tail_begin(&r_[k], &s_[k], &tails[k]);
                zk_tail_pre_a(pk, &tails[k]);
                zk_tail_pre_b(pk, &tails[k]);
                zk_tail_pre_2(pk, &tails[k]);
            }
        });
    });
    const std::function<void()> pre_ready = [&] { if (pre_task.valid()) pre_task.get(); };
    const std::function<int()> wmap = [&] { return zk_groth16_witness_map_batch(ctx, r, count, z_dev, wm.p); };
    const std::function<int()> none = [] { return ZK_OK; };
    int rc = ZK_OK;
    for (size_t k0 = 0; k0 < count && rc == ZK_OK; k0 += chunk)
        rc = prove_chunk(ctx, pk, r, std::min(chunk, count - k0), (const char*)z_dev + k0 * m * 32, (const char*)wm.p + k0 * D * 32,
                         k0 == 0 ? wmap : none, pre_ready, tails.data() + k0, proofs_out + k0 * 192);
    return rc;
}

}

extern "C" int zk_groth16_prove_batch_dev(zk_ctx* ctx, const zk_pk* pk, const zk_r1cs* r, size_t count, const void* z_dev, const zk_fr* r_,
                                          const zk_fr* s_, uint8_t* proofs_out) {
    ZK_API_BEGIN(ctx)
    if (!ctx || !pk || !r || !count || !z_dev || !r_ || !s_ || !proofs_out) return ZK_ERR_ARG;
    size_t chunk;
    ZK_TRY(batch_plan(ctx, pk, r, count, &chunk));
    return run_batch(ctx, pk, r, count, chunk, z_dev, r_, s_, proofs_out);
    ZK_API_END
}

extern "C" int zk_groth16_prove_batch(zk_ctx* ctx, const zk_pk* pk, const zk_r1cs* r, size_t count, const zk_fr* z_host, const zk_fr* r_,
                                      const zk_fr* s_, uint8_t* proofs_out) {
    ZK_API_BEGIN(ctx)
    if (!ctx || !pk || !r || !count || !z_host || !r_ || !s_ || !proofs_out) return ZK_ERR_ARG;
    size_t chunk;
    ZK_TRY(batch_plan(ctx, pk, r, count, &chunk));
    const size_t m = r->ni + r->nw;
    CallMem z{ctx};
    ZK_HIP(ctx, hipMalloc(&z.p, count * m * 32));
    ZK_TRY(zk_xfer_h2d(ctx, z.p, z_host, count * m * 32, zk_host_is_pinned(z_host)));
    return run_batch(ctx, pk, r, count, chunk, z.p, r_, s_, proofs_out);
    ZK_API_END
}
```

zk-mpc_amd/csrc/groth16_int.hpp:

```cpp
#pragma once
#include "devutil.cuh"
#include "hostgroup.hpp"
#include "hostfield64.hpp"
#include "internal.hpp"
#include "../../include/zkmpc_hip.h"
#include <algorithm>
#include <chrono>
#include <cstring>
#include <functional>
#include <future>
#include <memory>
#include <mutex>
#include <vector>

struct zk_r1cs {
    size_t nc = 0, ni = 0, nw = 0;
    uint32_t log_d = 0;
    struct Mat {
        uint32_t* row_ptr = nullptr;
        uint32_t* col = nullptr;
        uint32_t* coeff = nullptr;
        size_t nnz = 0;
        bool all_one = false;
        std::vector<uint32_t> h_row_ptr, h_col;
        std::vector<zk::Fr> h_coeff;
    } m[3];
};

struct zk_pk {
    zk_bases *a = nullptr, *b_g1 = nullptr, *b_g2 = nullptr, *h = nullptr, *l = nullptr, *gamma_abc = nullptr;
    zk_bases* l_pad = nullptr;
    bool points_in_subgroup = false;
    uint32_t mul_levels = 0;
    zk::Affine<zk::G1Field> alpha_g1, beta_g1, delta_g1, a0, b0_g1;
    zk::Affine<zk::G2Field> beta_g2, delta_g2, gamma_g2, b0_g2;
    mutable std::mutex e_alpha_beta_mu;
    mutable bool have_e_alpha_beta = false;
    mutable uint32_t e_alpha_beta[144];
};

struct ZkPresort {
    ZkMsmJob job;
    const zk_pk* pk = nullptr;
    const void* z = nullptr;
    bool front = false;
    const zk_r1cs* r = nullptr;
    void* h = nullptr;
    ZkMsmJob jobh;
    hipEvent_t wm_done = nullptr;
    bool begun = false;
    ZkMsmJob j1, j2, j3;
    bool chained = false;
    ~ZkPresort() { if (wm_done) (void)hipEventDestroy(wm_done); }
};

int zk_prover_streams(zk_ctx* ctx, size_t k);
int zk_groth16_run_msms(zk_ctx* ctx, const zk_pk* pk, const zk_r1cs* r, const void* z, const void* h_in, void* h_scratch,
                        zk_g1_projective out_g1[4], zk_g2_projective* out_g2, const std::function<void()>& after_abc = nullptr);
int zk_pk_make_l_pad(zk_ctx* ctx, zk_pk* pk);
int zk_pk_precompute(zk_ctx* ctx, zk_pk* pk);
int zk_groth16_witness_map_batch(zk_ctx* ctx, const zk_r1cs* r, size_t count, const void* z, void* abc);
int zk_groth16_key_matches(zk_ctx* ctx, const zk_pk* pk, const zk_r1cs* r);
int zk_next_z_drop(zk_ctx* ctx, bool drain);

struct ZkG16Jobs {
    struct Job {
        const zk_bases* tab;
        size_t off;
        const char* scal;
        size_t n;
    } j[5];
    size_t m, D;
    bool l_shared;
    ZkG16Jobs(const zk_pk* pk, const zk_r1cs* r, const void* z, const void* h, bool pad_l = true) : m(r->ni + r->nw), D((size_t)1 << r->log_d) {
        const size_t nvars = m - 1;
        const char *z1 = z ? (const char*)z + 32 : nullptr, *zw = z ? (const char*)z + r->ni * 32 : nullptr;
        l_shared = pad_l && pk->l_pad && pk->l_pad->n == nvars + 1 && (pk->l_pad->pre != nullptr) == (pk->a->pre != nullptr) &&
                   pk->l_pad->c_pre == pk->a->c_pre && pk->l_pad->pre_levels == pk->a->pre_levels;
        j[0] = {pk->b_g2, 1, z1, nvars};
        j[1] = {pk->a, 1, z1, nvars};
        j[2] = {pk->b_g1, 1, z1, nvars};
        j[3] = l_shared ? Job{pk->l_pad, 1, z1, nvars} : Job{pk->l, 0, zw, r->nw};
        j[4] = {pk->h, 0, (const char*)h, std::min(pk->h->n, D)};
    }
    int prepare(zk_ctx* ctx, int k, ZkMsmJob* job, ZkMsmSlot slot0, size_t multi = 0) const {
        if (!multi) return zk_msm_prepare(ctx, job, j[k].tab, j[k].off, j[k].scal, j[k].n, slot0 + k);
        return zk_msm_prepare_multi(ctx, job, j[k].tab, j[k].off, j[k].scal, j[k].n, k == 4 ? D : m, multi, slot0 + k);
    }
    int sort_z(zk_ctx* ctx, ZkMsmJob* const* J, hipStream_t st, ZkMsmSlot slot0, size_t multi = 0, bool have0 = false) const {
        for (int k = have0 ? 1 : 0; k < 4; k++) ZK_TRY(prepare(ctx, k, J[k], slot0, multi));
        if (!have0) ZK_TRY(zk_msm_enqueue_sort(ctx, J[0], st, nullptr));
        ZK_TRY(zk_msm_enqueue_sort(ctx, J[1], st, J[0]));
        const ZkMsmJob* lender = J[0]->c == J[1]->c ? J[0] : J[1];
        ZK_TRY(zk_msm_enqueue_sort(ctx, J[2], st, lender));
        return l_shared ? zk_msm_enqueue_sort(ctx, J[3], st, lender) : ZK_OK;
    }
};

struct ZkTail {
    using X1 = zk::XYZZ<zk::Fq64Field>;
    uint32_t rw[8], sw[8];
    X1 r_g1, r_s_delta, s_g1;
    zk::XYZZ<zk::Fq264Field> s_g2;
    X1 g_a, s_g_a, r_g1_b;
    zk::Affine<zk::Fq264Field> b_aff;
};
void zk_tail_begin(const zk_fr* r, const zk_fr* s, ZkTail* t);
void zk_tail_pre_a(const zk_pk* pk, ZkTail* t);
void zk_tail_pre_b(const zk_pk* pk, ZkTail* t);
void zk_tail_pre_2(const zk_pk* pk, ZkTail* t);
void zk_tail_chain_a(const zk_pk* pk, ZkTail* t, const zk_g1_projective& a_sum);
void zk_tail_chain_b(const zk_pk* pk, ZkTail* t, const zk_g1_projective& b1_sum);
void zk_tail_chain_2(const zk_pk* pk, ZkTail* t, const zk_g2_projective& b2_sum);
void zk_tail_finish(const ZkTail& t, const zk_g1_projective& h_sum, const zk_g1_projective& l_sum, uint8_t proof[192]);

class ZkProofTail {
    zk_ctx* ctx;
    const zk_pk* pk;
    ZkTail t;
    ZkTask<void> pre_a, pre_b, pre_2;
    ZkTask<void> chain_a, chain_b, chain_g2;

   public:
    ZkProofTail(zk_ctx* c, const zk_pk* pk, const zk_fr* r_, const zk_fr* s_);
    void abc_ready(const zk_g1_projective& a_sum, const zk_g1_projective& b1_sum, const zk_g2_projective& b2_sum);
    void join();
    void finish(const zk_g1_projective& h_sum, const zk_g1_projective& l_sum, uint8_t proof[192]);
};

namespace zk {
template <class F>
inline int first_point(zk_ctx* ctx, const zk_bases* b, Affine<F>* out) {
    if (!b || b->n == 0) { *out = aff_inf<F>(); return ZK_OK; }
    uint32_t w[2 * F::WORDS];
    ZK_HIP(ctx, hipMemcpy(w, b->dev, sizeof w, hipMemcpyDeviceToHost));
    *out = aff_load<F>(w);
    return ZK_OK;
}

}
```

zk-mpc_amd/csrc/groth16_key.hip:

```cpp
#include "../../include/zkmpc_hip.h"
#include "groth16_int.hpp"

using namespace zk;

namespace {

Fr host_fr_from_u64(uint64_t v) {
    Fr t = fp_zero<FrParams>();
    t.l[0] = (uint32_t)(v & MASK29);
    t.l[1] = (uint32_t)((v >> 29) & MASK29);
    t.l[2] = (uint32_t)(v >> 58);
    return fp_canon_to_int<FrParams>(t);
}

Fr host_fr_pow(const Fr& a, uint64_t e) {
    Fr r = fp_one<FrParams>();
    bool started = false;
    for (int b = 63; b >= 0; b--) {
        if (started) r = fp_sqr<FrParams>(r);
        if ((e >> b) & 1) { r = started ? fp_mul<FrParams>(r, a) : a; started = true; }
    }
    return r;
}

void host_batch_inverse(std::vector<Fr>& v) {
    std::vector<Fr> pre(v.size());
    Fr run = fp_one<FrParams>();
    for (size_t i = 0; i < v.size(); i++) {
        pre[i] = run;
        if (!fp_is_zero<FrParams>(v[i])) run = fp_mul<FrParams>(run, v[i]);
    }
    Fr inv = fp_inv<FrParams>(run);
    for (size_t i = v.size(); i-- > 0;) {
        if (fp_is_zero<FrParams>(v[i])) continue;
        Fr t = fp_mul<FrParams>(inv, pre[i]);
        inv = fp_mul<FrParams>(inv, v[i]);
        v[i] = t;
    }
}

int upload_fr(zk_ctx* ctx, const std::vector<Fr>& v, const char* slot, void** dev) {
    std::vector<uint32_t> packed(v.size() * 8 + 8);
    for (size_t i = 0; i < v.size(); i++) fp_pack<FrParams>(&packed[8 * i], fp_int_to_ext<FrParams>(v[i]));
    ZK_TRY(zk_scratch(ctx, slot, v.size() * 32 + 32, dev));
    ZK_HIP(ctx, hipMemcpyAsync(*dev, packed.data(), v.size() * 32, hipMemcpyHostToDevice, ctx->stream));
    ZK_HIP(ctx, hipStreamSynchronize(ctx->stream));
    return ZK_OK;
}

template <class F>
Affine<F> host_gen_mul(const Affine<F>& g, const Fr& k_int) {
    uint32_t kw[8];
    fp_pack<FrParams>(kw, fp_int_to_canon<FrParams>(k_int));
    return xyzz_to_affine<F>(xyzz_scalar_mul<F>(g, kw, 8));
}

Affine<G1Field> g1_gen() { return Affine<G1Field>{fp_const<FqParams>(FqParams::G1_GEN_X), fp_const<FqParams>(FqParams::G1_GEN_Y)}; }
Affine<G2Field> g2_gen() {
    return Affine<G2Field>{Fq2{fp_const<FqParams>(FqParams::G2_GEN_X0), fp_const<FqParams>(FqParams::G2_GEN_X1)},
                           Fq2{fp_const<FqParams>(FqParams::G2_GEN_Y0), fp_const<FqParams>(FqParams::G2_GEN_Y1)}};
}

}

int zk_pk_make_l_pad(zk_ctx* ctx, zk_pk* pk) {
    if (!pk->a || !pk->l || pk->l->n == 0 || pk->a->n <= pk->l->n) return ZK_OK;
    const size_t n = pk->a->n, front = n - pk->l->n, PW = 2 * G1Field::WORDS * 4;
    zk_bases* b = new zk_bases();
    b->group = 1;
    b->n = n;
    if (hipMalloc((void**)&b->dev, n * PW) != hipSuccess) { delete b; (void)hipGetLastError(); return ZK_OK; }
    pk->l_pad = b;
    ZK_HIP(ctx, hipMemsetAsync(b->dev, 0, front * PW, ctx->stream));
    ZK_HIP(ctx, hipMemcpyAsync((char*)b->dev + front * PW, pk->l->dev, pk->l->n * PW, hipMemcpyDeviceToDevice, ctx->stream));
    ZK_HIP(ctx, hipStreamSynchronize(ctx->stream));
    return zk_bases_precompute_levels(ctx, b, pk->mul_levels);
}

int zk_pk_precompute(zk_ctx* ctx, zk_pk* pk) {
    pk->mul_levels = pk->a ? zk_mul_levels_for_key(ctx, pk->a->n) : 0;
    for (zk_bases* q : {pk->a, pk->b_g1, pk->b_g2, pk->h, pk->l}) ZK_TRY(zk_bases_precompute_levels(ctx, q, pk->mul_levels));
    return zk_pk_make_l_pad(ctx, pk);
}
extern "C" uint32_t zk_pk_mul_levels(const zk_pk* pk) { return pk && pk->a ? pk->a->pre_levels : 0u; }
extern "C" int zk_msm_mul_levels(zk_ctx* ctx, int levels) {
    ZK_API_BEGIN(ctx)
    if (!ctx || levels < -1 || levels > (int)ZK_MSM_MAX_LEVELS) return ZK_ERR_ARG;
    ctx->mul_levels = levels;
    return ZK_OK;
    ZK_API_END
}

extern "C" int zk_pk_free(zk_ctx* ctx, zk_pk* pk) {
    ZK_API_BEGIN(ctx)
    if (!pk) return ZK_OK;
    zk_presort_free(ctx);
    zk_bases* all[7] = {pk->a, pk->b_g1, pk->b_g2, pk->h, pk->l, pk->gamma_abc, pk->l_pad};
    for (auto* b : all) zk_bases_free(ctx, b);
    delete pk;
    return ZK_OK;
    ZK_API_END
}

extern "C" int zk_pk_upload(zk_ctx* ctx, const zk_pk_host* h, zk_pk** out) {
    ZK_API_BEGIN(ctx)
    if (!ctx || !h || !out) return ZK_ERR_ARG;
    zk_pk* pk = new zk_pk();
    int rc = zk_bases_upload_g1(ctx, h->a_query, h->a_len, &pk->a);
    if (rc == ZK_OK) rc = zk_bases_upload_g1(ctx, h->b_g1_query, h->b_g1_len, &pk->b_g1);
    if (rc == ZK_OK) rc = zk_bases_upload_g2(ctx, h->b_g2_query, h->b_g2_len, &pk->b_g2);
    if (rc == ZK_OK) rc = zk_bases_upload_g1(ctx, h->h_query, h->h_len, &pk->h);
    if (rc == ZK_OK) rc = zk_bases_upload_g1(ctx, h->l_query, h->l_len, &pk->l);
    if (rc == ZK_OK) rc = zk_pk_precompute(ctx, pk);
    if (rc != ZK_OK) { zk_pk_free(ctx, pk); return rc; }
    pk->alpha_g1 = host_aff_from_abi<G1Field>((const uint64_t*)&h->alpha_g1);
    pk->beta_g1 = host_aff_from_abi<G1Field>((const uint64_t*)&h->beta_g1);
    pk->delta_g1 = host_aff_from_abi<G1Field>((const uint64_t*)&h->delta_g1);
    pk->beta_g2 = host_aff_from_abi<G2Field>((const uint64_t*)&h->beta_g2);
    pk->delta_g2 = host_aff_from_abi<G2Field>((const uint64_t*)&h->delta_g2);
    pk->gamma_g2 = aff_inf<G2Field>();
    pk->a0 = h->a_len ? host_aff_from_abi<G1Field>((const uint64_t*)&h->a_query[0]) : aff_inf<G1Field>();
    pk->b0_g1 = h->b_g1_len ? host_aff_from_abi<G1Field>((const uint64_t*)&h->b_g1_query[0]) : aff_inf<G1Field>();
    pk->b0_g2 = h->b_g2_len ? host_aff_from_abi<G2Field>((const uint64_t*)&h->b_g2_query[0]) : aff_inf<G2Field>();
    *out = pk;
    return ZK_OK;
    ZK_API_END
}

extern "C" size_t zk_pk_query_len(const zk_pk* pk, int which) {
    if (!pk) return 0;
    const zk_bases* all[6] = {pk->a, pk->b_g1, pk->b_g2, pk->h, pk->l, pk->gamma_abc};
    return (which >= 0 && which < 6 && all[which]) ? all[which]->n : 0;
}
extern "C" const zk_bases* zk_pk_query_bases(const zk_pk* pk, int which) {
    if (!pk || which < 0 || which > 5) return nullptr;
    const zk_bases* all[6] = {pk->a, pk->b_g1, pk->b_g2, pk->h, pk->l, pk->gamma_abc};
    return all[which];
}
extern "C" int zk_pk_download_g1(zk_ctx* ctx, const zk_pk* pk, int which, size_t off, size_t n, zk_g1_affine* out) {
    ZK_API_BEGIN(ctx)
    if (!pk || which == 2 || which < 0 || which > 5) return ZK_ERR_ARG;
    const zk_bases* all[6] = {pk->a, pk->b_g1, pk->b_g2, pk->h, pk->l, pk->gamma_abc};
    return zk_bases_download_g1(ctx, all[which], off, n, out);
    ZK_API_END
}
extern "C" int zk_pk_download_g2(zk_ctx* ctx, const zk_pk* pk, int which, size_t off, size_t n, zk_g2_affine* out) {
    ZK_API_BEGIN(ctx)
    if (!pk || which != 2) return ZK_ERR_ARG;
    return zk_bases_download_g2(ctx, pk->b_g2, off, n, out);
    ZK_API_END
}
extern "C" int zk_pk_vk_g1(const zk_pk* pk, int which, zk_g1_affine* out) {
    ZK_API_BEGIN_NOCTX
    if (!pk || !out || which < 0 || which > 2) return ZK_ERR_ARG;
    const Affine<G1Field>* v[3] = {&pk->alpha_g1, &pk->beta_g1, &pk->delta_g1};
    host_aff_to_abi<G1Field>((uint64_t*)out, *v[which]);
    return ZK_OK;
    ZK_API_END
}
extern "C" int zk_pk_vk_g2(const zk_pk* pk, int which, zk_g2_affine* out) {
    ZK_API_BEGIN_NOCTX
    if (!pk || !out || which < 0 || which > 2) return ZK_ERR_ARG;
    const Affine<G2Field>* v[3] = {&pk->beta_g2, &pk->delta_g2, &pk->gamma_g2};
    host_aff_to_abi<G2Field>((uint64_t*)out, *v[which]);
    return ZK_OK;
    ZK_API_END
}

extern "C" int zk_groth16_setup(zk_ctx* ctx, const zk_r1cs* r, const zk_fr* alpha_, const zk_fr* beta_, const zk_fr* gamma_,
                                const zk_fr* delta_, const zk_fr* tau_, const zk_fr* g1_k, const zk_fr* g2_k, zk_pk** out) {
    ZK_API_BEGIN(ctx)
    if (!ctx || !r || !alpha_ || !beta_ || !gamma_ || !delta_ || !tau_ || !g1_k || !g2_k || !out) return ZK_ERR_ARG;
    auto ld = [](const zk_fr* x) { return fp_ext_to_int<FrParams>(host_load_ext<FrParams>(x->l)); };
    const Fr alpha = ld(alpha_), beta = ld(beta_), gamma = ld(gamma_), delta = ld(delta_), t = ld(tau_);
    const Fr one = fp_one<FrParams>();
    const size_t D = (size_t)1 << r->log_d, nc = r->nc, ni = r->ni;
    const size_t nvars = (ni - 1) + r->nw;
    if (fp_is_zero<FrParams>(gamma) || fp_is_zero<FrParams>(delta)) ZK_FAIL(ctx, ZK_ERR_ARG, "setup: gamma/delta must be non-zero");

    Fr w = fp_const<FrParams>(FrParams::TWO_ADIC_ROOT);
    for (uint32_t i = 0; i < (uint32_t)FR_TWO_ADICITY - r->log_d; i++) w = fp_sqr<FrParams>(w);
    const Fr size_inv = fp_inv<FrParams>(host_fr_from_u64(D));
    const Fr zt = fp_sub<FrParams>(host_fr_pow(t, D), one);
    if (fp_is_zero<FrParams>(zt)) ZK_FAIL(ctx, ZK_ERR_ARG, "setup: tau lies in the evaluation domain");

    std::vector<Fr> u(D), den(D);
    {
        Fr l = fp_mul<FrParams>(zt, size_inv), rr = one;
        for (size_t i = 0; i < D; i++) {
            den[i] = fp_sub<FrParams>(t, rr);
            u[i] = l;
            l = fp_mul<FrParams>(l, w);
            rr = fp_mul<FrParams>(rr, w);
        }
        host_batch_inverse(den);
        for (size_t i = 0; i < D; i++) u[i] = fp_mul<FrParams>(u[i], den[i]);
        den.clear(); den.shrink_to_fit();
    }
    std::vector<Fr> a(nvars + 1, fp_zero<FrParams>()), b(nvars + 1, fp_zero<FrParams>()), c(nvars + 1, fp_zero<FrParams>());
    for (size_t i = 0; i < ni; i++) a[i] = u[nc + i];
    std::vector<Fr>* abc[3] = {&a, &b, &c};
    for (int k = 0; k < 3; k++) {
        const auto& m = r->m[k];
        auto& dst = *abc[k];
        for (size_t i = 0; i < nc; i++)
            for (uint32_t e = m.h_row_ptr[i]; e < m.h_row_ptr[i + 1]; e++) {
                Fr term = m.all_one ? u[i] : fp_mul<FrParams>(u[i], m.h_coeff[e]);
                dst[m.h_col[e]] = fp_add<FrParams>(dst[m.h_col[e]], term);
            }
    }
    u.clear(); u.shrink_to_fit();
    const Fr gamma_inv = fp_inv<FrParams>(gamma), delta_inv = fp_inv<FrParams>(delta);
    std::vector<Fr> gamma_abc(ni), l(nvars + 1 - ni);
    for (size_t i = 0; i <= nvars; i++) {
        Fr s = fp_add<FrParams>(fp_add<FrParams>(fp_mul<FrParams>(beta, a[i]), fp_mul<FrParams>(alpha, b[i])), c[i]);
        if (i < ni) gamma_abc[i] = fp_mul<FrParams>(s, gamma_inv);
        else l[i - ni] = fp_mul<FrParams>(s, delta_inv);
    }
    c.clear(); c.shrink_to_fit();
    std::vector<Fr> hq(D - 1);
    {
        Fr p = fp_mul<FrParams>(zt, delta_inv);
        for (size_t i = 0; i + 1 < D; i++) { hq[i] = p; p = fp_mul<FrParams>(p, t); }
    }

    zk_pk* pk = new zk_pk();
    void* dev;
    int rc = upload_fr(ctx, a, "setup_scalars", &dev);
    if (rc == ZK_OK) rc = zk_fixed_base_g1_dev(ctx, g1_k, dev, a.size(), &pk->a);
    if (rc == ZK_OK) rc = upload_fr(ctx, b, "setup_scalars", &dev);
    if (rc == ZK_OK) rc = zk_fixed_base_g1_dev(ctx, g1_k, dev, b.size(), &pk->b_g1);
    if (rc == ZK_OK) rc = zk_fixed_base_g2_dev(ctx, g2_k, dev, b.size(), &pk->b_g2);
    if (rc == ZK_OK) rc = upload_fr(ctx, hq, "setup_scalars", &dev);
    if (rc == ZK_OK) rc = zk_fixed_base_g1_dev(ctx, g1_k, dev, hq.size(), &pk->h);
    if (rc == ZK_OK) rc = upload_fr(ctx, l, "setup_scalars", &dev);
    if (rc == ZK_OK) rc = zk_fixed_base_g1_dev(ctx, g1_k, dev, l.size(), &pk->l);
    if (rc == ZK_OK) rc = upload_fr(ctx, gamma_abc, "setup_scalars", &dev);
    if (rc == ZK_OK) rc = zk_fixed_base_g1_dev(ctx, g1_k, dev, gamma_abc.size(), &pk->gamma_abc);
    if (rc == ZK_OK) rc = zk_pk_precompute(ctx, pk);
    if (rc != ZK_OK) { zk_pk_free(ctx, pk); return rc; }
    pk->points_in_subgroup = true;

    const Fr k1 = ld(g1_k), k2 = ld(g2_k);
    const Affine<G1Field> g1 = host_gen_mul<G1Field>(g1_gen(), k1);
    const Affine<G2Field> g2 = host_gen_mul<G2Field>(g2_gen(), k2);
    pk->alpha_g1 = host_gen_mul<G1Field>(g1, alpha);
    pk->beta_g1 = host_gen_mul<G1Field>(g1, beta);
    pk->delta_g1 = host_gen_mul<G1Field>(g1, delta);
    pk->beta_g2 = host_gen_mul<G2Field>(g2, beta);
    pk->delta_g2 = host_gen_mul<G2Field>(g2, delta);
    pk->gamma_g2 = host_gen_mul<G2Field>(g2, gamma);
    rc = first_point<G1Field>(ctx, pk->a, &pk->a0);
    if (rc == ZK_OK) rc = first_point<G1Field>(ctx, pk->b_g1, &pk->b0_g1);
    if (rc == ZK_OK) rc = first_point<G2Field>(ctx, pk->b_g2, &pk->b0_g2);
    if (rc != ZK_OK) { zk_pk_free(ctx, pk); return rc; }
    *out = pk;
    return ZK_OK;
    ZK_API_END
}
```

zk-mpc_amd/csrc/groth16_pipeline.hip:

```cpp
#include "../../include/zkmpc_hip.h"
#include "groth16_int.hpp"
#include <chrono>

using namespace zk;

void zk_presort_free(zk_ctx* ctx) {
    if (!ctx || !ctx->presort) return;
    ZkPresort* p = ctx->presort;
    ctx->presort = nullptr;
    if (ctx->aux.size()) (void)hipStreamSynchronize(ctx->aux[0]);
    if (p->front || p->begun) {
        if (ctx->acc_stream) (void)hipStreamSynchronize(ctx->acc_stream);
        (void)hipStreamSynchronize(ctx->stream);
    }
    delete p;
}

int zk_next_z_drop(zk_ctx* ctx, bool drain) {
    if (drain) {
        zk_presort_free(ctx);
        if (ctx->copy_stream) ZK_HIP(ctx, hipStreamSynchronize(ctx->copy_stream));
    }
    ctx->next_z = nullptr;
    ctx->next_z_host = nullptr;
    ctx->next_z_dev = nullptr;
    ctx->next_z_pk = ctx->next_z_r = nullptr;
    ctx->next_z_m = 0;
    return ZK_OK;
}

int zk_groth16_key_matches(zk_ctx* ctx, const zk_pk* pk, const zk_r1cs* r) {
    const size_t n = r->ni + r->nw;
    if (!pk->a || !pk->b_g1 || !pk->b_g2 || !pk->l || !pk->h || r->ni < 1 || pk->a->n != n || pk->b_g1->n != n || pk->b_g2->n != n ||
        pk->l->n != r->nw)
        ZK_FAIL(ctx, ZK_ERR_ARG, "groth16: proving key does not match the constraint system");
    return ZK_OK;
}

int zk_prover_streams(zk_ctx* ctx, size_t k) {
    while (ctx->aux.size() < k) {
        hipStream_t st;
        ZK_HIP(ctx, zk_stream_create(&st, true));
        ctx->aux.push_back(st);
    }
    if (!ctx->acc_stream) ZK_HIP(ctx, zk_stream_create(&ctx->acc_stream, false));
    return ZK_OK;
}

int zk_groth16_run_msms(zk_ctx* ctx, const zk_pk* pk, const zk_r1cs* r, const void* z, const void* h_in, void* h_scratch,
                        zk_g1_projective out_g1[4], zk_g2_projective* out_g2, const std::function<void()>& after_abc) {
    const auto t_enter = std::chrono::steady_clock::now();
    ZK_TRY(zk_groth16_key_matches(ctx, pk, r));
    const ZkG16Jobs T(pk, r, z, h_in ? h_in : h_scratch);
    const size_t D = T.D, nvars = T.j[0].n;
    const bool l_shared = T.l_shared;
    ZK_TRY(zk_prover_streams(ctx, 1));
    hipStream_t s_sort = ctx->aux[0], s_acc = ctx->acc_stream;
    struct Events {
        hipEvent_t e0 = nullptr, e1 = nullptr;
        ~Events() { if (e0) (void)hipEventDestroy(e0); if (e1) (void)hipEventDestroy(e1); }
    } evs;
    ZK_HIP(ctx, hipEventCreateWithFlags(&evs.e0, hipEventDisableTiming));
    ZK_HIP(ctx, hipEventCreateWithFlags(&evs.e1, hipEventDisableTiming));
    const hipEvent_t e0 = evs.e0, e1 = evs.e1;
    ZK_HIP(ctx, hipEventRecord(e0, ctx->stream));
    ZkMsmJob own[5];
    ZkMsmJob* J[5] = {&own[0], &own[1], &own[2], &own[3], &own[4]};
    ZkPresort* pre = ctx->presort;
    ctx->presort = nullptr;
    std::unique_ptr<ZkPresort> pre_owner(pre);
    const bool presorted = pre && pre->pk == pk && pre->z == z && pre->job.n == nvars && (!pre->begun || (h_in && pre->r == r));
    const bool fronted = presorted && pre->front && !h_in && pre->r == r && pre->h == h_scratch;
    if (pre && !presorted) {
        pre_owner.release();
        ctx->presort = pre;
        zk_presort_free(ctx);
        pre = nullptr;
    }
    const bool begun = presorted && pre->begun && h_in && pre->r == r;
    const bool chained = fronted && pre->chained;
    if (presorted) J[0] = &pre->job;
    if (fronted) J[4] = &pre->jobh;
    if (begun || chained) { J[1] = &pre->j1; J[2] = &pre->j2; J[3] = &pre->j3; }
    if (!fronted) ZK_HIP(ctx, hipStreamWaitEvent(s_sort, e0, 0));
    const bool have_z_jobs = begun || chained;
    int rc = have_z_jobs ? ZK_OK : T.sort_z(ctx, J, s_sort, ZK_SLOT_G16, 0, presorted);
    ZkPhaseTimer tm(ctx);
    if (fronted) {
        ZK_HIP(ctx, hipStreamWaitEvent(s_acc, pre->wm_done, 0));
    } else {
        if (rc == ZK_OK && !h_in) {
            tm.begin("witness_map");
            rc = zk_groth16_witness_map_dev(ctx, r, z, h_scratch);
            tm.end();
        }
        if (rc == ZK_OK) rc = T.prepare(ctx, 4, J[4], ZK_SLOT_G16);
        if (rc == ZK_OK) {
            ZK_HIP(ctx, hipEventRecord(e1, ctx->stream));
            ZK_HIP(ctx, hipStreamWaitEvent(s_acc, e1, 0));
            rc = zk_msm_enqueue_sort(ctx, J[4], ctx->stream, nullptr);
        }
    }
    if (rc == ZK_OK && !l_shared && !have_z_jobs) {
        ZK_HIP(ctx, hipStreamWaitEvent(s_sort, e1, 0));
        rc = zk_msm_enqueue_sort(ctx, J[3], s_sort, nullptr);
    }
    const bool small_jobs = !begun && D <= ((size_t)1 << 16);
    auto job_stream = [&](int k) -> hipStream_t { return k == 0 ? s_acc : ((k & 1) ? s_sort : ctx->stream); };
    ZkMsmJob* g1jobs[4] = {J[1], J[2], J[3], J[4]};
    const bool grouped = chained || (small_jobs && rc == ZK_OK && zk_msm_group_ok(g1jobs, 4));
    for (int k = 0; k < 5 && rc == ZK_OK && !chained; k++) {
        if (grouped && k != 0) continue;
        if (!begun || k == 4) rc = zk_msm_enqueue_accum(ctx, J[k], small_jobs ? job_stream(k) : s_acc);
    }
    if (grouped && !chained && rc == ZK_OK) rc = zk_msm_enqueue_accum_group(ctx, g1jobs, 4, s_sort);
    for (int k = 0; k < 5 && rc == ZK_OK && !chained; k++) {
        hipStream_t rs = small_jobs ? job_stream(k) : ((k & 1) == 0 ? s_sort : ctx->stream);
        if (begun && k == 0) continue;
        if (grouped && k != 0) continue;
        rc = zk_msm_enqueue_reduce(ctx, J[k], rs);
    }
    if (grouped && !chained && rc == ZK_OK) rc = zk_msm_enqueue_reduce_group(ctx, g1jobs, 4, s_sort);
    bool front_enqueued = false;
    if (rc == ZK_OK && ctx->next_z && !h_in && l_shared) {
        const void* zn = ctx->next_z;
        ctx->next_z = nullptr;
        std::unique_ptr<ZkPresort> nf(new ZkPresort());
        nf->pk = pk; nf->z = zn; nf->r = r; nf->h = h_scratch; nf->front = true;
        if (zn == ctx->next_z_dev && ctx->next_z_ready) {
            ZK_HIP(ctx, hipStreamWaitEvent(s_acc, ctx->next_z_ready, 0));
            ZK_HIP(ctx, hipStreamWaitEvent(ctx->stream, ctx->next_z_ready, 0));
        }
        for (int k = 0; k < 4; k++)
            if (J[k]->reduce_done) ZK_HIP(ctx, hipStreamWaitEvent(s_acc, J[k]->reduce_done, 0));
        const ZkG16Jobs N(pk, r, zn, h_scratch);
        rc = N.prepare(ctx, 0, &nf->job, ZK_SLOT_G16);
        if (rc == ZK_OK) rc = zk_msm_enqueue_sort(ctx, &nf->job, s_acc, nullptr);
        if (rc == ZK_OK) rc = zk_groth16_witness_map_dev(ctx, r, zn, h_scratch);
        if (rc == ZK_OK) {
            ZK_HIP(ctx, hipEventCreateWithFlags(&nf->wm_done, hipEventDisableTiming));
            ZK_HIP(ctx, hipEventRecord(nf->wm_done, ctx->stream));
            if (J[4]->accum_done) ZK_HIP(ctx, hipStreamWaitEvent(ctx->stream, J[4]->accum_done, 0));
            if (J[4]->reduce_done) ZK_HIP(ctx, hipStreamWaitEvent(ctx->stream, J[4]->reduce_done, 0));
            rc = N.prepare(ctx, 4, &nf->jobh, ZK_SLOT_G16);
            if (rc == ZK_OK) rc = zk_msm_enqueue_sort(ctx, &nf->jobh, ctx->stream, nullptr);
        }
        if (rc == ZK_OK && grouped && ctx->chain_fronts) {
            const int par = (ctx->front_parity ^= 1);
            nf->job.pin = {ZK_PIN_FRONT, (uint32_t)par};
            nf->j1.pin = {ZK_PIN_FRONT_GROUP, (uint32_t)par};
            ZkMsmJob* nz[4] = {&nf->job, &nf->j1, &nf->j2, &nf->j3};
            rc = N.sort_z(ctx, nz, s_acc, ZK_SLOT_G16, 0, true);
            ZkMsmJob* ng[4] = {&nf->j1, &nf->j2, &nf->j3, &nf->jobh};
            if (rc == ZK_OK && zk_msm_group_ok(ng, 4)) {
                rc = zk_msm_enqueue_accum(ctx, &nf->job, s_acc);
                if (rc == ZK_OK) rc = zk_msm_enqueue_accum_group(ctx, ng, 4, s_sort);
                if (rc == ZK_OK) rc = zk_msm_enqueue_reduce(ctx, &nf->job, s_acc);
                if (rc == ZK_OK) rc = zk_msm_enqueue_reduce_group(ctx, ng, 4, s_sort);
                nf->chained = rc == ZK_OK;
            }
            if (rc != ZK_OK) {
                ctx->presort = nf.release();
                zk_presort_free(ctx);
            }
        }
        if (rc == ZK_OK) { ctx->presort = nf.release(); front_enqueued = true; }
    }
    ctx->next_z = nullptr;
    if (ctx->profiling) {
        auto& t = ctx->timers["host.enqueue"];
        t.ms += std::chrono::duration<float, std::milli>(std::chrono::steady_clock::now() - t_enter).count();
        t.count += 1;
    }
    void* outs[5] = {out_g2, &out_g1[2], &out_g1[3], &out_g1[1], &out_g1[0]};
    if (grouped && rc == ZK_OK) {
        void* gouts[4] = {outs[1], outs[2], outs[3], outs[4]};
        ZkTask<int> g1fin = zk_async(ctx, [&] { (void)hipSetDevice(ctx->device); return zk_msm_finish_many(ctx, g1jobs, gouts, 4); });
        rc = zk_msm_finish(ctx, J[0], outs[0]);
        const int rc1 = g1fin.get();
        if (rc == ZK_OK) rc = rc1;
        if (rc == ZK_OK && after_abc) after_abc();
    } else {
        for (int k = 0; k < 5 && rc == ZK_OK; k++) {
            rc = zk_msm_finish(ctx, J[k], outs[k]);
            if (k == 2 && rc == ZK_OK && after_abc) after_abc();
        }
    }
    if (!front_enqueued) {
        (void)hipStreamSynchronize(s_sort);
        (void)hipStreamSynchronize(s_acc);
        (void)hipStreamSynchronize(ctx->stream);
    }
    tm.resolve();
    return rc;
}


extern "C" int zk_groth16_hint_next_dev(zk_ctx* ctx, const void* z_next_dev) {
    ZK_API_BEGIN(ctx)
    if (!ctx) return ZK_ERR_ARG;
    ctx->next_z = z_next_dev;
    return ZK_OK;
    ZK_API_END
}

extern "C" int zk_groth16_chain_fronts(zk_ctx* ctx, int on) {
    ZK_API_BEGIN(ctx)
    if (!ctx) return ZK_ERR_ARG;
    ctx->chain_fronts = on != 0;
    return ZK_OK;
    ZK_API_END
}

extern "C" int zk_groth16_msms_presort_dev(zk_ctx* ctx, const zk_pk* pk, const zk_r1cs* r, const void* z) {
    ZK_API_BEGIN(ctx)
    if (!ctx || !pk || !r || !z) return ZK_ERR_ARG;
    zk_presort_free(ctx);
    ZK_TRY(zk_groth16_key_matches(ctx, pk, r));
    ZK_TRY(zk_prover_streams(ctx, 1));
    hipEvent_t e0;
    ZK_HIP(ctx, hipEventCreateWithFlags(&e0, hipEventDisableTiming));
    ZK_HIP(ctx, hipEventRecord(e0, ctx->stream));
    ZK_HIP(ctx, hipStreamWaitEvent(ctx->aux[0], e0, 0));
    (void)hipEventDestroy(e0);
    std::unique_ptr<ZkPresort> p(new ZkPresort());
    p->pk = pk;
    p->z = z;
    ZK_TRY(ZkG16Jobs(pk, r, z, nullptr).prepare(ctx, 0, &p->job, ZK_SLOT_G16));
    ZK_TRY(zk_msm_enqueue_sort(ctx, &p->job, ctx->aux[0], nullptr));
    ctx->presort = p.release();
    return ZK_OK;
    ZK_API_END
}

extern "C" int zk_groth16_msms_begin_dev(zk_ctx* ctx, const zk_pk* pk, const zk_r1cs* r, const void* z) {
    ZK_API_BEGIN(ctx)
    if (!ctx || !pk || !r || !z) return ZK_ERR_ARG;
    zk_presort_free(ctx);
    ZK_TRY(zk_groth16_key_matches(ctx, pk, r));
    ZK_TRY(zk_prover_streams(ctx, 1));
    hipStream_t s_sort = ctx->aux[0], s_acc = ctx->acc_stream;
    hipEvent_t e0;
    ZK_HIP(ctx, hipEventCreateWithFlags(&e0, hipEventDisableTiming));
    ZK_HIP(ctx, hipEventRecord(e0, ctx->stream));
    ZK_HIP(ctx, hipStreamWaitEvent(s_sort, e0, 0));
    ZK_HIP(ctx, hipStreamWaitEvent(s_acc, e0, 0));
    (void)hipEventDestroy(e0);
    std::unique_ptr<ZkPresort> p(new ZkPresort());
    p->pk = pk; p->z = z; p->r = r; p->begun = true;
    const ZkG16Jobs T(pk, r, z, nullptr);
    ZkMsmJob* J[4] = {&p->job, &p->j1, &p->j2, &p->j3};
    int rc = T.sort_z(ctx, J, s_sort, ZK_SLOT_G16);
    if (rc == ZK_OK && !T.l_shared) rc = zk_msm_enqueue_sort(ctx, J[3], s_sort, nullptr);
    for (int k = 0; k < 4 && rc == ZK_OK; k++) rc = zk_msm_enqueue_accum(ctx, J[k], s_acc);
    if (rc == ZK_OK) rc = zk_msm_enqueue_reduce(ctx, J[0], s_sort);
    if (rc != ZK_OK) {
        (void)hipStreamSynchronize(s_sort);
        (void)hipStreamSynchronize(s_acc);
        return rc;
    }
    ctx->presort = p.release();
    return ZK_OK;
    ZK_API_END
}

extern "C" int zk_groth16_msms_dev(zk_ctx* ctx, const zk_pk* pk, const zk_r1cs* r, const void* z, const void* h,
                                   zk_g1_projective out_g1[4], zk_g2_projective* out_g2) {
    ZK_API_BEGIN(ctx)
    if (!ctx || !pk || !r || !z || !h || !out_g1 || !out_g2) return ZK_ERR_ARG;
    return zk_groth16_run_msms(ctx, pk, r, z, h, nullptr, out_g1, out_g2);
    ZK_API_END
}
```

zk-mpc_amd/csrc/groth16_prove.hip:

```cpp
#include "../../include/zkmpc_hip.h"
#include <string.h>
#include "groth16_int.hpp"

using namespace zk;

namespace {
using H1 = Fq64Field;
using H2 = Fq264Field;
using X1 = XYZZ<H1>;
X1 mul1(const zk_pk* pk, const X1& p, const uint32_t* k) { return pk->points_in_subgroup ? host64_scalar_mul_glv(p, k) : host64_scalar_mul<H1>(p, k); }
template <class H, class G>
XYZZ<H> coeff(const XYZZ<H>& initial, const Affine<G>& q0, const void* acc, const Affine<G>& vk_param) {
    return xyzz_madd<H>(xyzz_add<H>(xyzz_madd<H>(initial, aff_to_host64<G>(q0)), host64_proj_from_abi<H>((const uint64_t*)acc)), aff_to_host64<G>(vk_param));
}
}

void zk_tail_begin(const zk_fr* r, const zk_fr* s, ZkTail* t) {
    fr_abi_to_canon_words(r->l, t->rw);
    fr_abi_to_canon_words(s->l, t->sw);
}
void zk_tail_pre_a(const zk_pk* pk, ZkTail* t) {
    t->r_g1 = mul1(pk, xyzz_from_affine<H1>(aff_to_host64<G1Field>(pk->delta_g1)), t->rw);
    t->r_s_delta = mul1(pk, t->r_g1, t->sw);
}
void zk_tail_pre_b(const zk_pk* pk, ZkTail* t) { t->s_g1 = mul1(pk, xyzz_from_affine<H1>(aff_to_host64<G1Field>(pk->delta_g1)), t->sw); }
void zk_tail_pre_2(const zk_pk* pk, ZkTail* t) { t->s_g2 = host64_scalar_mul<H2>(xyzz_from_affine<H2>(aff_to_host64<G2Field>(pk->delta_g2)), t->sw); }
void zk_tail_chain_a(const zk_pk* pk, ZkTail* t, const zk_g1_projective& a_sum) {
    t->g_a = coeff<H1>(t->r_g1, pk->a0, &a_sum, pk->alpha_g1);
    t->s_g_a = mul1(pk, t->g_a, t->sw);
}
void zk_tail_chain_b(const zk_pk* pk, ZkTail* t, const zk_g1_projective& b1_sum) {
    t->r_g1_b = mul1(pk, coeff<H1>(t->s_g1, pk->b0_g1, &b1_sum, pk->beta_g1), t->rw);
}
void zk_tail_chain_2(const zk_pk* pk, ZkTail* t, const zk_g2_projective& b2_sum) {
    t->b_aff = xyzz_to_affine<H2>(coeff<H2>(t->s_g2, pk->b0_g2, &b2_sum, pk->beta_g2));
}
void zk_tail_finish(const ZkTail& t, const zk_g1_projective& h_sum, const zk_g1_projective& l_sum, uint8_t proof[192]) {
    X1 g_c = xyzz_add<H1>(t.s_g_a, t.r_g1_b);
    g_c = xyzz_add<H1>(g_c, xyzz_neg<H1>(t.r_s_delta));
    g_c = xyzz_add<H1>(g_c, host64_proj_from_abi<H1>((const uint64_t*)&l_sum));
    g_c = xyzz_add<H1>(g_c, host64_proj_from_abi<H1>((const uint64_t*)&h_sum));
    g1_serialize(aff_from_host64<G1Field>(xyzz_to_affine<H1>(t.g_a)), proof);
    g2_serialize(aff_from_host64<G2Field>(t.b_aff), proof + 48);
    g1_serialize(aff_from_host64<G1Field>(xyzz_to_affine<H1>(g_c)), proof + 144);
}

ZkProofTail::ZkProofTail(zk_ctx* c, const zk_pk* pk_, const zk_fr* r_, const zk_fr* s_) : ctx(c), pk(pk_) {
    zk_tail_begin(r_, s_, &t);
    pre_a = zk_async(ctx, [this] { zk_tail_pre_a(pk, &t); });
    pre_b = zk_async(ctx, [this] { zk_tail_pre_b(pk, &t); });
    pre_2 = zk_async(ctx, [this] { zk_tail_pre_2(pk, &t); });
}

void ZkProofTail::abc_ready(const zk_g1_projective& a_sum, const zk_g1_projective& b1_sum, const zk_g2_projective& b2_sum) {
    chain_a = zk_async(ctx, [this, a_sum] { pre_a.wait(); zk_tail_chain_a(pk, &t, a_sum); });
    chain_b = zk_async(ctx, [this, b1_sum] { pre_b.wait(); zk_tail_chain_b(pk, &t, b1_sum); });
    chain_g2 = zk_async(ctx, [this, b2_sum] { pre_2.wait(); zk_tail_chain_2(pk, &t, b2_sum); });
}

void ZkProofTail::join() {
    if (chain_a.valid()) chain_a.get();
    if (chain_b.valid()) chain_b.get();
    if (chain_g2.valid()) chain_g2.get();
    if (pre_a.valid()) pre_a.wait();
    if (pre_b.valid()) pre_b.wait();
    if (pre_2.valid()) pre_2.wait();
}

void ZkProofTail::finish(const zk_g1_projective& h_sum, const zk_g1_projective& l_sum, uint8_t proof[192]) {
    join();
    zk_tail_finish(t, h_sum, l_sum, proof);
}

extern "C" int zk_groth16_prove_dev(zk_ctx* ctx, const zk_pk* pk, const zk_r1cs* r, const void* z, const zk_fr* r_, const zk_fr* s_,
                                    uint8_t proof[192]) {
    ZK_API_BEGIN(ctx)
    if (!ctx || !pk || !r || !z || !r_ || !s_ || !proof) return ZK_ERR_ARG;
    const size_t D = (size_t)1 << r->log_d;
    void* h;
    ZK_TRY(zk_scratch(ctx, "prove_h", D * 32, &h));
    zk_g1_projective m1[4];
    zk_g2_projective m2;
    ZkProofTail tail(ctx, pk, r_, s_);
    const int rc_msm = zk_groth16_run_msms(ctx, pk, r, z, nullptr, h, m1, &m2, [&] { tail.abc_ready(m1[2], m1[3], m2); });
    const auto t_tail = std::chrono::steady_clock::now();
    tail.join();
    ZK_TRY(rc_msm);
    tail.finish(m1[0], m1[1], proof);
    if (ctx->profiling) {
        auto& t = ctx->timers["host.tail"];
        t.ms += std::chrono::duration<float, std::milli>(std::chrono::steady_clock::now() - t_tail).count();
        t.count += 1;
    }
    return ZK_OK;
    ZK_API_END
}

extern "C" int zk_groth16_prove_queued(zk_ctx* ctx, const zk_pk* pk, const zk_r1cs* r, const zk_fr* z_host, const zk_fr* r_,
                                       const zk_fr* s_, const zk_fr* z_next_host, uint8_t proof[192]) {
    ZK_API_BEGIN(ctx)
    if (!ctx || !pk || !r || !z_host) return ZK_ERR_ARG;
    const size_t m = r->ni + r->nw;
    void* z;
    if (ctx->next_z_host == z_host && ctx->next_z_dev && ctx->next_z_pk == pk && ctx->next_z_r == r && ctx->next_z_m == m) {
        z = ctx->next_z_dev;
        ctx->z_slot ^= 1;
        ZK_HIP(ctx, hipStreamWaitEvent(ctx->stream, ctx->next_z_ready, 0));
        ZK_TRY(zk_next_z_drop(ctx, false));
    } else {
        ZK_TRY(zk_next_z_drop(ctx, true));
        ZK_TRY(zk_scratch(ctx, ctx->z_slot ? "prove_z1" : "prove_z0", m * 32, &z));
        ZK_TRY(zk_xfer_h2d(ctx, z, z_host, m * 32, zk_host_is_pinned(z_host)));
    }
    if (z_next_host) {
        if (!ctx->copy_stream) ZK_HIP(ctx, zk_stream_create(&ctx->copy_stream, false));
        if (!ctx->next_z_ready) ZK_HIP(ctx, hipEventCreateWithFlags(&ctx->next_z_ready, hipEventDisableTiming));
        void* zn;
        ZK_TRY(zk_scratch(ctx, ctx->z_slot ? "prove_z0" : "prove_z1", m * 32, &zn));
        if (zk_host_is_pinned(z_next_host)) {
            ZK_HIP(ctx, hipMemcpyAsync(zn, z_next_host, m * 32, hipMemcpyHostToDevice, ctx->copy_stream));
            ZK_HIP(ctx, hipEventRecord(ctx->next_z_ready, ctx->copy_stream));
        } else {
            const char* src = (const char*)z_next_host;
            const ZkXferFill fill = [src](char* dst, size_t off, size_t len) { memcpy(dst, src + off, len); };
            ZK_TRY(zk_xfer_h2d_fn(ctx, zn, m * 32, fill, false, nullptr));
            hipStream_t xs;
            ZK_TRY(zk_xfer_stream(ctx, &xs));
            ZK_HIP(ctx, hipEventRecord(ctx->next_z_ready, xs));
        }
        ctx->next_z_host = z_next_host;
        ctx->next_z_dev = zn;
        ctx->next_z = zn;
        ctx->next_z_pk = pk; ctx->next_z_r = r; ctx->next_z_m = m;
    }
    return zk_groth16_prove_dev(ctx, pk, r, z, r_, s_, proof);
    ZK_API_END
}

extern "C" int zk_groth16_prove(zk_ctx* ctx, const zk_pk* pk, const zk_r1cs* r, const zk_fr* z_host, const zk_fr* r_, const zk_fr* s_,
                                uint8_t proof[192]) {
    ZK_API_BEGIN(ctx)
    return zk_groth16_prove_queued(ctx, pk, r, z_host, r_, s_, nullptr, proof);
    ZK_API_END
}
```

zk-mpc_amd/csrc/internal.hpp:

```cpp
#pragma once
#include "ctx.hpp"
#include "ec.cuh"
#include <stddef.h>
#include <stdint.h>
#include <atomic>
#include <functional>
#include <string>
#include <vector>

void zk_domains_free(zk_ctx* ctx);
void zk_presort_free(zk_ctx* ctx);
extern "C" int zk_comm_destroy(zk_ctx* ctx);
extern "C" int zk_fr_sum_parties_dev(zk_ctx* ctx, const void* gathered_dev, size_t n_parties, size_t n, void* out_dev);
int zk_ntt_launch(zk_ctx* ctx, void* buf_dev, uint32_t log_n, int inverse, int coset);
int zk_ntt_launch_batch(zk_ctx* ctx, void* const* bufs_dev, int count, uint32_t log_n, int inverse, int coset);
int zk_ntt_launch_strided(zk_ctx* ctx, void* base, size_t count, size_t stride, uint32_t log_n, int inverse, int coset, void* tmp = nullptr);
int zk_ntt_vanishing_inv(zk_ctx* ctx, uint32_t log_n, uint32_t out9[9]);

enum ZkLdsAttr { ZK_LDS_NTT, ZK_LDS_SORT_SMALL, ZK_LDS_SORT_SMALL_GROUP, ZK_LDS_SORT_GROUP, ZK_LDS_SHE, ZK_LDS_LINCOMB, ZK_LDS_COUNT };
static_assert(ZK_LDS_COUNT <= sizeof(zk_ctx::lds_attr_done), "zk_ctx::lds_attr_done is too short");

bool zk_fr_words_valid(const uint64_t l[4]);

int zk_graph_run(zk_ctx* ctx, const std::string& key, hipStream_t st, const std::function<int()>& enqueue);
int zk_vec_op_launch(zk_ctx* ctx, int op, const void* a, const void* b, void* out, size_t n);
int zk_vec_scale_launch(zk_ctx* ctx, const void* a, const uint32_t* k_int_form9, void* out, size_t n);
int zk_fr_vec_is_zero_launch(zk_ctx* ctx, const void* v, size_t n, int slot, const uint32_t** verdict);
int zk_fr_outer_q1_launch(zk_ctx* ctx, const void* s, const void* a, const void* b, const void* z, const void* rp, const void* tp,
                          const uint32_t* ka_int9, const uint32_t* kb_int9, const uint32_t* kc_int9, void* out, size_t n);
int zk_fr_lincomb_launch(zk_ctx* ctx, int terms, const void* const* ps, const size_t* ns, const uint32_t (*k_int_form9)[9], void* out, size_t n_out);
int zk_vec_sub_scale_launch(zk_ctx* ctx, const void* a, const void* b, const uint32_t* k_int_form9, void* out, size_t n);

struct zk_bases {
    int group = 1;
    size_t n = 0;
    uint32_t* dev = nullptr;
    bool owned = true;
    uint32_t* pre = nullptr;
    uint32_t c_pre = 0, W_pre = 0;
    uint32_t pre_stride = 0;
    uint32_t pre_levels = 0;
    std::string pre_note;
};
int zk_xfer_h2d(zk_ctx* ctx, void* dev, const void* host, size_t bytes, bool pinned = false);
int zk_xfer_d2h(zk_ctx* ctx, void* host, const void* dev, size_t bytes, bool pinned = false);
using ZkXferFill = std::function<void(char* dst, size_t off, size_t len)>;
using ZkXferDrain = std::function<void(const char* src, size_t off, size_t len)>;
int zk_xfer_h2d_fn(zk_ctx* ctx, void* dev, size_t bytes, const ZkXferFill& fill, bool fence_ctx,
                   const std::function<int(size_t, size_t, hipStream_t)>* after_round);
int zk_xfer_d2h_fn(zk_ctx* ctx, const void* dev, size_t bytes, const ZkXferDrain& drain);
int zk_xfer_stream(zk_ctx* ctx, hipStream_t* st);
void zk_xfer_free(zk_ctx* ctx);
bool zk_host_is_pinned(const void* host);
struct ZkAffineLayout { size_t stride, off_x, off_y, off_inf; };
int zk_bases_upload_host(zk_ctx* ctx, int group, const void* host, size_t n, const ZkAffineLayout* layout, zk_bases** out);
int zk_bases_alloc_dev(zk_ctx* ctx, int group, size_t n, zk_bases** out);
int zk_bases_import_launch(zk_ctx* ctx, zk_bases* b, const void* raw_dev, hipStream_t st);
struct ZkHostTable {
    int group = 1;
    const void* host = nullptr;
    size_t stride = 0, off_x = 0, off_y = 0, off_inf = SIZE_MAX, off_tag = SIZE_MAX;
    uint8_t tag_public = 0;
};
struct ZkBasesLease {
    zk_ctx* const ctx;
    const zk_bases* b = nullptr;
    bool temporary = false;
    bool verify = false;
    uint32_t* raw_tmp = nullptr;
    void* stage = nullptr;
    const void* entry = nullptr;
    explicit ZkBasesLease(zk_ctx* c) : ctx(c) {}
    ~ZkBasesLease();
    ZkBasesLease(const ZkBasesLease&) = delete;
    ZkBasesLease& operator=(const ZkBasesLease&) = delete;
};
int zk_bases_cache_get(zk_ctx* ctx, const ZkHostTable& t, size_t n, ZkBasesLease* out);
int zk_bases_cache_verify(zk_ctx* ctx, ZkBasesLease* l, const ZkHostTable& t, size_t n, bool* same);
int zk_bases_cache_replace(zk_ctx* ctx, ZkBasesLease* l);
int zk_msm_table_run(zk_ctx* ctx, const ZkHostTable& t, size_t n_table, int n_lanes, const void* const* scalars_dev, size_t n, void* const* outs,
                     uint64_t scalars_fp = 0);
void zk_msm_spec_drop(zk_ctx* ctx);
int zk_side_stream(zk_ctx* ctx, hipStream_t* out);
void zk_msm_spec_forget(zk_ctx* ctx, const zk_bases* b);
void zk_msm_spec_fft_begin(zk_ctx* ctx, const void* dev, size_t N, int kind);
void zk_msm_spec_fft_end(zk_ctx* ctx, size_t N, int kind, const std::function<uint64_t(size_t)>& fp_of);
uint64_t zk_scalars_fingerprint(const void* fr, size_t n);
void zk_msm_spec_free(zk_ctx* ctx);
int zk_prover_streams(zk_ctx* ctx, size_t k);
int zk_bases_cache_poll(zk_ctx* ctx);
void zk_bases_cache_free(zk_ctx* ctx);
extern "C" int zk_bases_free(zk_ctx* ctx, zk_bases* b);
constexpr size_t ZK_PRECOMP_MIN_POINTS = 256;
extern "C" int zk_bases_precompute(zk_ctx* ctx, zk_bases* b);
constexpr uint32_t ZK_MSM_MAX_LEVELS = 3, ZK_MSM_MIN_LOG_NB = 6;
extern "C" uint32_t zk_msm_mul_levels_clamp(uint32_t c, uint32_t levels);
uint32_t zk_mul_levels_for_key(zk_ctx* ctx, size_t n);
int zk_bases_precompute_levels(zk_ctx* ctx, zk_bases* b, uint32_t levels);
uint32_t zk_precompute_windows(size_t n);
int zk_bases_precompute_auto(zk_ctx* ctx, zk_bases* b);
struct ZkPrecompJob {
    zk_bases* b = nullptr;
    uint32_t c = 0, W = 0, wide_words = 0;
    uint32_t *packed = nullptr, *wide = nullptr, *xy = nullptr, *scr = nullptr;
    int phase = -1;
    uint32_t w = 1;
    size_t pos = 0, budget = 0;
    hipError_t err = hipSuccess;
};
int zk_bases_precompute_begin(zk_ctx* ctx, zk_bases* b, size_t budget_bytes, ZkPrecompJob** out);
hipError_t zk_bases_precompute_step(ZkPrecompJob* j, hipStream_t st, bool* more);
void zk_bases_precompute_finish(ZkPrecompJob* j, bool keep);
int zk_msm_run(zk_ctx* ctx, const zk_bases* bases, size_t base_offset, const void* scalars_dev, size_t n,
               void* out_host_projective);

struct ZkPhaseTimer {
    zk_ctx* ctx;
    hipStream_t stream;
    std::vector<std::pair<std::string, std::pair<hipEvent_t, hipEvent_t>>> ev;
    bool enabled;
    bool resolved = false;
    explicit ZkPhaseTimer(zk_ctx* c, hipStream_t st = nullptr);
    ~ZkPhaseTimer();
    void begin(const char* name);
    void end();
    void resolve();
};

enum ZkPinKind : uint8_t {
    ZK_PIN_OF_SLOT = 0,
    ZK_PIN_MSM_SLOT,
    ZK_PIN_MSM_GROUP,
    ZK_PIN_BATCH_JOB,
    ZK_PIN_AHEAD,
    ZK_PIN_FRONT,
    ZK_PIN_FRONT_GROUP,
    ZK_PIN_MULTI_Z,
    ZK_PIN_STRIDED_UPLOAD,
    ZK_PIN_INV_TOTALS,
    ZK_PIN_ZERO_VERDICTS,
};

enum ZkMsmSlot : int {
    ZK_SLOT_RUN = 0,
    ZK_SLOT_G16 = 1,
    ZK_SLOT_AHEAD = 6,
    ZK_SLOT_G16_BATCH = 8,
    ZK_SLOT_END = 13,
};
constexpr int ZK_SLOT_G16_COUNT = 5, ZK_SLOT_AHEAD_COUNT = 2;
static_assert(ZK_SLOT_RUN + 1 <= ZK_SLOT_G16 && ZK_SLOT_G16 + ZK_SLOT_G16_COUNT <= ZK_SLOT_AHEAD &&
              ZK_SLOT_AHEAD + ZK_SLOT_AHEAD_COUNT <= ZK_SLOT_G16_BATCH && ZK_SLOT_G16_BATCH + ZK_SLOT_G16_COUNT <= ZK_SLOT_END,
              "the MSM scratch slot ranges overlap");

struct ZkMsmJob {
    int group = 1, slot = 0;
    ZkPin pin = {ZK_PIN_OF_SLOT, 0};
    size_t n = 0, max_segs = 0, max_heavy = 0;
    uint32_t c = 0, W = 0, NB = 0, seg = 0;
    uint16_t off[65] = {0};
    uint32_t Wb = 0;
    uint32_t log_nb = 0, nout = 0;
    uint32_t M = 0, red_win = 1, lvl_stride = 0;
    uint32_t n_tab = 0, tab_off = 0;
    uint32_t stride = 0;
    const uint32_t* bases_dev = nullptr;
    const void* scalars = nullptr;
    hipStream_t stream = nullptr;
    hipStream_t sort_stream = nullptr, accum_stream = nullptr;
    hipEvent_t sort_done = nullptr;
    hipEvent_t accum_done = nullptr;
    hipEvent_t reduce_done = nullptr;
    uint32_t* hw = nullptr;
    uint32_t *sorted = nullptr, *order = nullptr, *ctr = nullptr;
    void *desc = nullptr, *heavy = nullptr, *heavy2 = nullptr;
    size_t max_heavy2 = 0, max_heavy_segs = 0, max_groups = 0;
    std::vector<ZkPhaseTimer*> timers;
    size_t mcount = 0, mn = 0, mstride = 0;
    ~ZkMsmJob();
};
// ... 51 lines not shown
```

zk-mpc_amd/csrc/r1cs.hip:

```cpp
#include "../../include/zkmpc_hip.h"
#include "groth16_int.hpp"

using namespace zk;

namespace {

uint32_t domain_log(size_t num_coeffs) {
    uint32_t lg = 0;
    while (((size_t)1 << lg) < num_coeffs) lg++;
    return lg;
}

__global__ void __launch_bounds__(256)
k_spmv(const uint32_t* row_ptr, const uint32_t* col, const uint32_t* coeff, int all_one, const void* z, size_t nc,
       size_t n_copy, size_t D, void* out) {
    for (size_t r = blockIdx.x * (size_t)blockDim.x + threadIdx.x; r < D; r += (size_t)gridDim.x * blockDim.x) {
        Fr acc = fp_zero<FrParams>();
        if (r < nc) {
            uint32_t lo = row_ptr[r], hi = row_ptr[r + 1];
            for (uint32_t k = lo; k < hi; k++) {
                Fr v = fr_load(z, col[k]);
                if (!all_one) v = fr_mul(v, fr_load(coeff, k));
                acc = fr_add(acc, v);
            }
// ... 108 lines not shown
    ZK_API_END
}

extern "C" int zk_r1cs_mul_chain(zk_ctx* ctx, size_t n, zk_r1cs** out) {
    ZK_API_BEGIN(ctx)
    if (!ctx || !out || n == 0 || n > ((size_t)1 << 27)) return ZK_ERR_ARG;
    auto idx = [n](size_t j) -> uint32_t { return j <= n ? (uint32_t)(2 + j) : 1u; };
    std::vector<uint32_t> rp(n + 1), ca(n), cb(n), cc(n);
    for (size_t i = 0; i <= n; i++) rp[i] = (uint32_t)i;
    for (size_t i = 0; i < n; i++) { ca[i] = idx(i); cb[i] = idx(i + 1); cc[i] = idx(i + 2); }
    zk_fr one_ext;
    host_store_ext<FrParams>(one_ext.l, fp_int_to_ext<FrParams>(fp_one<FrParams>()));
    std::vector<zk_fr> ones(n, one_ext);
    zk_r1cs_host h;
    h.num_constraints = n; h.num_instance = 2; h.num_witness = n + 1;
    h.a_row_ptr = h.b_row_ptr = h.c_row_ptr = rp.data();
    h.a_col = ca.data(); h.b_col = cb.data(); h.c_col = cc.data();
    h.a_coeff = h.b_coeff = h.c_coeff = ones.data();
    return zk_r1cs_upload(ctx, &h, out);
    ZK_API_END
}

extern "C" int zk_mul_chain_assignment_dev(zk_ctx* ctx, size_t n, const zk_fr* w0, const zk_fr* w1, void* z_dev) {
    ZK_API_BEGIN(ctx)
    if (!ctx || !w0 || !w1 || !z_dev || n == 0) return ZK_ERR_ARG;
    std::vector<Fr> w(n + 2);
    w[0] = fp_ext_to_int<FrParams>(host_load_ext<FrParams>(w0->l));
    w[1] = fp_ext_to_int<FrParams>(host_load_ext<FrParams>(w1->l));
    for (size_t i = 0; i < n; i++) w[i + 2] = fp_mul<FrParams>(w[i], w[i + 1]);
    std::vector<uint32_t> packed((n + 3) * 8);
    fp_pack<FrParams>(&packed[0], fp_int_to_ext<FrParams>(fp_one<FrParams>()));
    fp_pack<FrParams>(&packed[8], fp_int_to_ext<FrParams>(w[n + 1]));
    for (size_t j = 0; j <= n; j++) fp_pack<FrParams>(&packed[8 * (2 + j)], fp_int_to_ext<FrParams>(w[j]));
    ZK_HIP(ctx, hipMemcpyAsync(z_dev, packed.data(), packed.size() * 4, hipMemcpyHostToDevice, ctx->stream));
    ZK_HIP(ctx, hipStreamSynchronize(ctx->stream));
    return ZK_OK;
    ZK_API_END
}


extern "C" int zk_groth16_witness_map_pre_dev(zk_ctx* ctx, const zk_r1cs* r, const void* z, int include_instance, void* a,
                                              void* b, void* c) {
    ZK_API_BEGIN(ctx)
    if (!ctx || !r || !z || !a || !b || !c) return ZK_ERR_ARG;
    ZK_TRY(spmv(ctx, r, 0, z, include_instance ? r->ni : 0, a));
    ZK_TRY(spmv(ctx, r, 1, z, 0, b));
    ZK_TRY(spmv(ctx, r, 2, z, 0, c));
    void* v[3] = {a, b, c};
    ZK_TRY(zk_ntt_launch_batch(ctx, v, 3, r->log_d, 1, 0));
    return zk_ntt_launch_batch(ctx, v, 2, r->log_d, 0, 1);
    ZK_API_END
}

extern "C" int zk_groth16_witness_map_post_dev(zk_ctx* ctx, const zk_r1cs* r, void* ab, const void* c) {
    ZK_API_BEGIN(ctx)
    if (!ctx || !r || !ab || !c) return ZK_ERR_ARG;
    uint32_t zinv[9];
    ZK_TRY(zk_ntt_vanishing_inv(ctx, r->log_d, zinv));
    ZK_TRY(zk_ntt_launch(ctx, ab, r->log_d, 1, 1));
    return zk_vec_sub_scale_launch(ctx, ab, c, zinv, ab, (size_t)1 << r->log_d);
    ZK_API_END
}

int zk_groth16_witness_map_batch(zk_ctx* ctx, const zk_r1cs* r, size_t count, const void* z, void* abc) {
    const size_t D = (size_t)1 << r->log_d, m = r->ni + r->nw, total = count * D;
    char* a = (char*)abc;
    char *b = a + total * 32, *c = b + total * 32, *tmp = c + total * 32;
    const unsigned g = zk_grid(total, 256);
    for (int which = 0; which < 3; which++) {
        const auto& mt = r->m[which];
        hipLaunchKernelGGL(k_spmv_multi, g, 256, 0, ctx->stream, mt.row_ptr, mt.col, mt.coeff, mt.all_one ? 1 : 0, z, m, r->nc,
                           which == 0 ? r->ni : (size_t)0, r->log_d, total, (void*)(which == 0 ? a : which == 1 ? b : c));
    }
    ZK_HIP(ctx, hipGetLastError());
    ZK_TRY(zk_ntt_launch_strided(ctx, a, 3 * count, D, r->log_d, 1, 0, tmp));
    ZK_TRY(zk_ntt_launch_strided(ctx, a, 2 * count, D, r->log_d, 0, 1, tmp));
    ZK_TRY(zk_vec_op_launch(ctx, ZK_OP_MUL, a, b, a, total));
    uint32_t zinv[9];
    ZK_TRY(zk_ntt_vanishing_inv(ctx, r->log_d, zinv));
    ZK_TRY(zk_ntt_launch_strided(ctx, a, count, D, r->log_d, 1, 1, tmp));
    return zk_vec_sub_scale_launch(ctx, a, c, zinv, a, total);
}

extern "C" int zk_groth16_witness_map_dev(zk_ctx* ctx, const zk_r1cs* r, const void* z, void* h) {
    ZK_API_BEGIN(ctx)
    if (!ctx || !r || !z || !h) return ZK_ERR_ARG;
    size_t D = (size_t)1 << r->log_d;
    void *b, *c;
    ZK_TRY(zk_scratch(ctx, "wm_b", D * 32, &b));
    ZK_TRY(zk_scratch(ctx, "wm_c", D * 32, &c));
    ZK_TRY(zk_groth16_witness_map_pre_dev(ctx, r, z, 1, h, b, c));
    ZK_TRY(zk_vec_op_launch(ctx, ZK_OP_MUL, h, b, h, D));
    return zk_groth16_witness_map_post_dev(ctx, r, h, c);
    ZK_API_END
}
```

Baseline: 70.49 million constraints/s.

## Fold quotient division and C term into evaluation-form H and L keys

Adds setup-time key tables (h_eval, l_eval_pad plus a constant point) so the prover can MSM directly over the coset evaluations of A*B. This skips the C spmv, its NTTs, the inverse coset NTT and the sub-scale step in the witness map. The C contribution and the vanishing-polynomial inverse are folded into the L and H bases at setup. The cost is extra setup work and GPU memory for two more precomputed tables, and the path is gated by an env var and a free-memory check.

```diff
diff --git a/bindings/hip_ffi.rs b/bindings/hip_ffi.rs
--- a/bindings/hip_ffi.rs
+++ b/bindings/hip_ffi.rs
@@ -305,6 +305,7 @@
     pub fn zk_pk_query_bases(pk: *const ZkPk, which: i32) -> *const ZkBases;
     pub fn zk_msm_mul_levels(ctx: *mut ZkCtx, levels: i32) -> i32;
     pub fn zk_pk_mul_levels(pk: *const ZkPk) -> u32;
+    pub fn zk_pk_eval_h(pk: *const ZkPk, r1cs: *const ZkR1cs) -> i32;
     pub fn zk_msm_mul_levels_clamp(window_bits: u32, levels: u32) -> u32;
     pub fn zk_pk_download_g1(ctx: *mut ZkCtx, pk: *const ZkPk, which: i32, offset: usize, n: usize, out: *mut ZkG1Affine) -> i32;
     pub fn zk_pk_download_g2(ctx: *mut ZkCtx, pk: *const ZkPk, which: i32, offset: usize, n: usize, out: *mut ZkG2Affine) -> i32;
diff --git a/include/zkmpc_hip.h b/include/zkmpc_hip.h
--- a/include/zkmpc_hip.h
+++ b/include/zkmpc_hip.h
@@ -169,6 +169,7 @@
 const zk_bases* zk_pk_query_bases(const zk_pk* pk, int which);
 int zk_msm_mul_levels(zk_ctx* ctx, int levels);
 uint32_t zk_pk_mul_levels(const zk_pk* pk);
+int zk_pk_eval_h(const zk_pk* pk, const zk_r1cs* r1cs);
 uint32_t zk_msm_mul_levels_clamp(uint32_t window_bits, uint32_t levels);
 int zk_pk_download_g1(zk_ctx* ctx, const zk_pk* pk, int which, size_t offset, size_t n, zk_g1_affine* out);
 int zk_pk_download_g2(zk_ctx* ctx, const zk_pk* pk, int which, size_t offset, size_t n, zk_g2_affine* out);
diff --git a/zk-mpc_amd/_lib.py b/zk-mpc_amd/_lib.py
--- a/zk-mpc_amd/_lib.py
+++ b/zk-mpc_amd/_lib.py
@@ -180,6 +180,7 @@
     "zk_pk_query_bases": (_P, [_P, _I]),
     "zk_msm_mul_levels": (_I, [_P, _I]),
     "zk_pk_mul_levels": (_U32, [_P]),
+    "zk_pk_eval_h": (_I, [_P, _P]),
     "zk_msm_mul_levels_clamp": (_U32, [_U32, _U32]),
     "zk_pk_download_g1": (_I, [_P, _P, _I, _SZ, _SZ, _P]),
     "zk_pk_download_g2": (_I, [_P, _P, _I, _SZ, _SZ, _P]),
diff --git a/zk-mpc_amd/api.py b/zk-mpc_amd/api.py
--- a/zk-mpc_amd/api.py
+++ b/zk-mpc_amd/api.py
@@ -874,6 +874,9 @@
     def mul_levels(self) -> int:
         return self.ctx.lib.zk_pk_mul_levels(self.h)
 
+    def eval_h(self, r1cs: "R1cs") -> bool:
+        return bool(self.ctx.lib.zk_pk_eval_h(self.h, r1cs.h))
+
     def query_len(self, name: str) -> int:
         return self.ctx.lib.zk_pk_query_len(self.h, self.QUERIES[name])
 
diff --git a/zk-mpc_amd/csrc/fixed_base.hip b/zk-mpc_amd/csrc/fixed_base.hip
--- a/zk-mpc_amd/csrc/fixed_base.hip
+++ b/zk-mpc_amd/csrc/fixed_base.hip
@@ -329,8 +329,13 @@
     if (!M) return 0;
     size_t mem_free = 0, mem_total = 0;
     if (hipMemGetInfo(&mem_free, &mem_total) != hipSuccess) { (void)hipGetLastError(); return 0; }
-    while (M && (size_t)(M + 1) * W * n * (4 * 256 + 96 + 192) > mem_free / 3) M--;
+    while (M && zk_key_tables_bytes(n, M, 4) > mem_free / 3) M--;
     return M;
+}
+size_t zk_key_tables_bytes(size_t n, uint32_t M, int g1_tables) {
+    if (n < ZK_PRECOMP_MIN_POINTS || !precompute_enabled_by_default()) return n * ((size_t)g1_tables * 96 + 192);
+    const uint32_t c = precompute_window_bits(n), W = (255 + c - 1) / c;
+    return (size_t)(M + 1) * W * n * ((size_t)g1_tables * 256 + 96 + 192);
 }
 int zk_bases_precompute_levels(zk_ctx* ctx, zk_bases* b, uint32_t levels) {
     if (!precompute_enabled_by_default() || !b || b->n < ZK_PRECOMP_MIN_POINTS) return ZK_OK;
diff --git a/zk-mpc_amd/csrc/groth16_batch.hip b/zk-mpc_amd/csrc/groth16_batch.hip
--- a/zk-mpc_amd/csrc/groth16_batch.hip
+++ b/zk-mpc_amd/csrc/groth16_batch.hip
@@ -67,7 +67,7 @@
             zk_tail_chain_a(pk, &tails[k], a[k]);
             zk_tail_chain_b(pk, &tails[k], b1[k]);
             zk_tail_chain_2(pk, &tails[k], b2[k]);
-            zk_tail_finish(tails[k], hs[k], l[k], proofs + k * 192);
+            zk_tail_finish(tails[k], hs[k], l[k], proofs + k * 192, T.l_const);
         }
     });
     return ZK_OK;
@@ -130,7 +130,7 @@
         });
     });
     const std::function<void()> pre_ready = [&] { if (pre_task.valid()) pre_task.get(); };
-    const std::function<int()> wmap = [&] { return zk_groth16_witness_map_batch(ctx, r, count, z_dev, wm.p); };
+    const std::function<int()> wmap = [&] { return ZkG16Jobs(pk, r, nullptr, nullptr).witness_map_batch(ctx, count, z_dev, wm.p); };
     const std::function<int()> none = [] { return ZK_OK; };
     int rc = ZK_OK;
     for (size_t k0 = 0; k0 < count && rc == ZK_OK; k0 += chunk)
diff --git a/zk-mpc_amd/csrc/groth16_int.hpp b/zk-mpc_amd/csrc/groth16_int.hpp
--- a/zk-mpc_amd/csrc/groth16_int.hpp
+++ b/zk-mpc_amd/csrc/groth16_int.hpp
@@ -6,6 +6,7 @@
 #include "../../include/zkmpc_hip.h"
 #include <algorithm>
 #include <chrono>
+#include <cstdlib>
 #include <cstring>
 #include <functional>
 #include <future>
@@ -30,6 +31,8 @@
 struct zk_pk {
     zk_bases *a = nullptr, *b_g1 = nullptr, *b_g2 = nullptr, *h = nullptr, *l = nullptr, *gamma_abc = nullptr;
     zk_bases* l_pad = nullptr;
+    zk_bases *h_eval = nullptr, *l_eval_pad = nullptr;
+    zk::Affine<zk::G1Field> l_eval_0;
     bool points_in_subgroup = false;
     uint32_t mul_levels = 0;
     zk::Affine<zk::G1Field> alpha_g1, beta_g1, delta_g1, a0, b0_g1;
@@ -59,7 +62,13 @@
                         zk_g1_projective out_g1[4], zk_g2_projective* out_g2, const std::function<void()>& after_abc = nullptr);
 int zk_pk_make_l_pad(zk_ctx* ctx, zk_pk* pk);
 int zk_pk_precompute(zk_ctx* ctx, zk_pk* pk);
+inline bool zk_g16_eval_h_enabled() {
+    static const bool on = [] { const char* e = getenv("ZK_G16_EVAL_H"); return !(e && *e && atoi(e) == 0); }();
+    return on;
+}
 int zk_groth16_witness_map_batch(zk_ctx* ctx, const zk_r1cs* r, size_t count, const void* z, void* abc);
+int zk_groth16_witness_map_eval_dev(zk_ctx* ctx, const zk_r1cs* r, const void* z, void* e);
+int zk_groth16_witness_map_eval_batch(zk_ctx* ctx, const zk_r1cs* r, size_t count, const void* z, void* abc);
 int zk_groth16_key_matches(zk_ctx* ctx, const zk_pk* pk, const zk_r1cs* r);
 int zk_next_z_drop(zk_ctx* ctx, bool drain);
 
@@ -72,16 +81,35 @@
     } j[5];
     size_t m, D;
     bool l_shared;
-    ZkG16Jobs(const zk_pk* pk, const zk_r1cs* r, const void* z, const void* h, bool pad_l = true) : m(r->ni + r->nw), D((size_t)1 << r->log_d) {
+    bool eval_h;
+    const zk::Affine<zk::G1Field>* l_const = nullptr;
+    const zk_r1cs* r;
+    ZkG16Jobs(const zk_pk* pk, const zk_r1cs* r_, const void* z, const void* h, bool pad_l = true, bool quotient_given = false)
+        : m(r_->ni + r_->nw), D((size_t)1 << r_->log_d), r(r_) {
         const size_t nvars = m - 1;
         const char *z1 = z ? (const char*)z + 32 : nullptr, *zw = z ? (const char*)z + r->ni * 32 : nullptr;
-        l_shared = pad_l && pk->l_pad && pk->l_pad->n == nvars + 1 && (pk->l_pad->pre != nullptr) == (pk->a->pre != nullptr) &&
-                   pk->l_pad->c_pre == pk->a->c_pre && pk->l_pad->pre_levels == pk->a->pre_levels;
+        auto like_a = [&](const zk_bases* t) {
+            return t && t->n == nvars + 1 && (t->pre != nullptr) == (pk->a->pre != nullptr) && t->c_pre == pk->a->c_pre && t->pre_levels == pk->a->pre_levels;
+        };
+        l_shared = pad_l && like_a(pk->l_pad);
+        eval_h = pad_l && !quotient_given && zk_g16_eval_h_enabled() && pk->h_eval && pk->h_eval->n == D && like_a(pk->l_eval_pad);
         j[0] = {pk->b_g2, 1, z1, nvars};
         j[1] = {pk->a, 1, z1, nvars};
         j[2] = {pk->b_g1, 1, z1, nvars};
         j[3] = l_shared ? Job{pk->l_pad, 1, z1, nvars} : Job{pk->l, 0, zw, r->nw};
         j[4] = {pk->h, 0, (const char*)h, std::min(pk->h->n, D)};
+        if (eval_h) {
+            l_shared = true;
+            j[3] = {pk->l_eval_pad, 1, z1, nvars};
+            j[4] = {pk->h_eval, 0, (const char*)h, D};
+            l_const = &pk->l_eval_0;
+        }
+    }
+    int witness_map(zk_ctx* ctx, const void* z, void* h) const {
+        return eval_h ? zk_groth16_witness_map_eval_dev(ctx, r, z, h) : zk_groth16_witness_map_dev(ctx, r, z, h);
+    }
+    int witness_map_batch(zk_ctx* ctx, size_t count, const void* z, void* abc) const {
+        return eval_h ? zk_groth16_witness_map_eval_batch(ctx, r, count, z, abc) : zk_groth16_witness_map_batch(ctx, r, count, z, abc);
     }
     int prepare(zk_ctx* ctx, int k, ZkMsmJob* job, ZkMsmSlot slot0, size_t multi = 0) const {
         if (!multi) return zk_msm_prepare(ctx, job, j[k].tab, j[k].off, j[k].scal, j[k].n, slot0 + k);
@@ -112,7 +140,8 @@
 void zk_tail_chain_a(const zk_pk* pk, ZkTail* t, const zk_g1_projective& a_sum);
 void zk_tail_chain_b(const zk_pk* pk, ZkTail* t, const zk_g1_projective& b1_sum);
 void zk_tail_chain_2(const zk_pk* pk, ZkTail* t, const zk_g2_projective& b2_sum);
-void zk_tail_finish(const ZkTail& t, const zk_g1_projective& h_sum, const zk_g1_projective& l_sum, uint8_t proof[192]);
+void zk_tail_finish(const ZkTail& t, const zk_g1_projective& h_sum, const zk_g1_projective& l_sum, uint8_t proof[192],
+                    const zk::Affine<zk::G1Field>* l_const = nullptr);
 
 class ZkProofTail {
     zk_ctx* ctx;
@@ -125,7 +154,7 @@
     ZkProofTail(zk_ctx* c, const zk_pk* pk, const zk_fr* r_, const zk_fr* s_);
     void abc_ready(const zk_g1_projective& a_sum, const zk_g1_projective& b1_sum, const zk_g2_projective& b2_sum);
     void join();
-    void finish(const zk_g1_projective& h_sum, const zk_g1_projective& l_sum, uint8_t proof[192]);
+    void finish(const zk_g1_projective& h_sum, const zk_g1_projective& l_sum, uint8_t proof[192], const zk::Affine<zk::G1Field>* l_const = nullptr);
 };
 
 namespace zk {
diff --git a/zk-mpc_amd/csrc/groth16_key.hip b/zk-mpc_amd/csrc/groth16_key.hip
--- a/zk-mpc_amd/csrc/groth16_key.hip
+++ b/zk-mpc_amd/csrc/groth16_key.hip
@@ -79,8 +79,13 @@
 
 int zk_pk_precompute(zk_ctx* ctx, zk_pk* pk) {
     pk->mul_levels = pk->a ? zk_mul_levels_for_key(ctx, pk->a->n) : 0;
-    for (zk_bases* q : {pk->a, pk->b_g1, pk->b_g2, pk->h, pk->l}) ZK_TRY(zk_bases_precompute_levels(ctx, q, pk->mul_levels));
+    for (zk_bases* q : {pk->a, pk->b_g1, pk->b_g2, pk->h, pk->l, pk->h_eval, pk->l_eval_pad}) ZK_TRY(zk_bases_precompute_levels(ctx, q, pk->mul_levels));
     return zk_pk_make_l_pad(ctx, pk);
+}
+extern "C" int zk_pk_eval_h(const zk_pk* pk, const zk_r1cs* r) {
+    ZK_API_BEGIN_NOCTX
+    return pk && r && pk->a && pk->h && pk->l && r->ni + r->nw == pk->a->n && ZkG16Jobs(pk, r, nullptr, nullptr).eval_h ? 1 : 0;
+    ZK_API_END
 }
 extern "C" uint32_t zk_pk_mul_levels(const zk_pk* pk) { return pk && pk->a ? pk->a->pre_levels : 0u; }
 extern "C" int zk_msm_mul_levels(zk_ctx* ctx, int levels) {
@@ -95,7 +100,7 @@
     ZK_API_BEGIN(ctx)
     if (!pk) return ZK_OK;
     zk_presort_free(ctx);
-    zk_bases* all[7] = {pk->a, pk->b_g1, pk->b_g2, pk->h, pk->l, pk->gamma_abc, pk->l_pad};
+    zk_bases* all[9] = {pk->a, pk->b_g1, pk->b_g2, pk->h, pk->l, pk->gamma_abc, pk->l_pad, pk->h_eval, pk->l_eval_pad};
     for (auto* b : all) zk_bases_free(ctx, b);
     delete pk;
     return ZK_OK;
@@ -209,7 +214,6 @@
                 dst[m.h_col[e]] = fp_add<FrParams>(dst[m.h_col[e]], term);
             }
     }
-    u.clear(); u.shrink_to_fit();
     const Fr gamma_inv = fp_inv<FrParams>(gamma), delta_inv = fp_inv<FrParams>(delta);
     std::vector<Fr> gamma_abc(ni), l(nvars + 1 - ni);
     for (size_t i = 0; i <= nvars; i++) {
@@ -223,6 +227,37 @@
         Fr p = fp_mul<FrParams>(zt, delta_inv);
         for (size_t i = 0; i + 1 < D; i++) { hq[i] = p; p = fp_mul<FrParams>(p, t); }
     }
+    bool eval_h = zk_g16_eval_h_enabled() && D >= 2;
+    if (eval_h) {
+        size_t mem_free = 0, mem_total = 0;
+        if (hipMemGetInfo(&mem_free, &mem_total) != hipSuccess) { (void)hipGetLastError(); mem_free = 0; }
+        eval_h = zk_key_tables_bytes(nvars + 1, zk_mul_levels_for_key(ctx, nvars + 1), 6) <= mem_free / 2;
+    }
+    std::vector<Fr> he, le;
+    if (eval_h) {
+        uint32_t zw[9];
+        ZK_TRY(zk_ntt_vanishing_inv(ctx, r->log_d, zw));
+        Fr zinv;
+        for (int i = 0; i < 9; i++) zinv.l[i] = zw[i];
+        const Fr k = fp_mul<FrParams>(zinv, delta_inv), t_top = host_fr_pow(t, D - 1);
+        std::vector<Fr> nv(nc);
+        Fr rr = one;
+        for (size_t i = 0; i < nc; i++) {
+            nv[i] = fp_mul<FrParams>(fp_mul<FrParams>(u[i], k), fp_sub<FrParams>(one, fp_mul<FrParams>(t_top, rr)));
+            rr = fp_mul<FrParams>(rr, w);
+        }
+        le.assign(nvars + 1, fp_zero<FrParams>());
+        for (size_t i = ni; i <= nvars; i++) le[i] = l[i - ni];
+        const auto& mc = r->m[2];
+        for (size_t i = 0; i < nc; i++)
+            for (uint32_t e = mc.h_row_ptr[i]; e < mc.h_row_ptr[i + 1]; e++)
+                le[mc.h_col[e]] = fp_add<FrParams>(le[mc.h_col[e]], mc.all_one ? nv[i] : fp_mul<FrParams>(nv[i], mc.h_coeff[e]));
+        he.assign(D, fp_zero<FrParams>());
+        const Fr q = fp_mul<FrParams>(t, fp_const<FrParams>(FrParams::GENERATOR_INV));
+        Fr p = fp_mul<FrParams>(zinv, fp_mul<FrParams>(zt, delta_inv));
+        for (size_t i = 0; i + 1 < D; i++) { he[i] = p; p = fp_mul<FrParams>(p, q); }
+    }
+    u.clear(); u.shrink_to_fit();
 
     zk_pk* pk = new zk_pk();
     void* dev;
@@ -237,6 +272,14 @@
     if (rc == ZK_OK) rc = zk_fixed_base_g1_dev(ctx, g1_k, dev, l.size(), &pk->l);
     if (rc == ZK_OK) rc = upload_fr(ctx, gamma_abc, "setup_scalars", &dev);
     if (rc == ZK_OK) rc = zk_fixed_base_g1_dev(ctx, g1_k, dev, gamma_abc.size(), &pk->gamma_abc);
+    if (eval_h) {
+        if (rc == ZK_OK) rc = upload_fr(ctx, he, "setup_scalars", &dev);
+        if (rc == ZK_OK) rc = zk_ntt_launch(ctx, dev, r->log_d, 1, 0);
+        if (rc == ZK_OK) rc = zk_fixed_base_g1_dev(ctx, g1_k, dev, D, &pk->h_eval);
+        if (rc == ZK_OK) rc = upload_fr(ctx, le, "setup_scalars", &dev);
+        if (rc == ZK_OK) rc = zk_fixed_base_g1_dev(ctx, g1_k, dev, le.size(), &pk->l_eval_pad);
+        if (rc == ZK_OK) rc = first_point<G1Field>(ctx, pk->l_eval_pad, &pk->l_eval_0);
+    }
     if (rc == ZK_OK) rc = zk_pk_precompute(ctx, pk);
     if (rc != ZK_OK) { zk_pk_free(ctx, pk); return rc; }
     pk->points_in_subgroup = true;
diff --git a/zk-mpc_amd/csrc/groth16_pipeline.hip b/zk-mpc_amd/csrc/groth16_pipeline.hip
--- a/zk-mpc_amd/csrc/groth16_pipeline.hip
+++ b/zk-mpc_amd/csrc/groth16_pipeline.hip
@@ -51,7 +51,7 @@
                         zk_g1_projective out_g1[4], zk_g2_projective* out_g2, const std::function<void()>& after_abc) {
     const auto t_enter = std::chrono::steady_clock::now();
     ZK_TRY(zk_groth16_key_matches(ctx, pk, r));
-    const ZkG16Jobs T(pk, r, z, h_in ? h_in : h_scratch);
+    const ZkG16Jobs T(pk, r, z, h_in ? h_in : h_scratch, true, h_in != nullptr);
     const size_t D = T.D, nvars = T.j[0].n;
     const bool l_shared = T.l_shared;
     ZK_TRY(zk_prover_streams(ctx, 1));
@@ -91,7 +91,7 @@
     } else {
         if (rc == ZK_OK && !h_in) {
             tm.begin("witness_map");
-            rc = zk_groth16_witness_map_dev(ctx, r, z, h_scratch);
+            rc = T.witness_map(ctx, z, h_scratch);
             tm.end();
         }
         if (rc == ZK_OK) rc = T.prepare(ctx, 4, J[4], ZK_SLOT_G16);
@@ -136,7 +136,7 @@
         const ZkG16Jobs N(pk, r, zn, h_scratch);
         rc = N.prepare(ctx, 0, &nf->job, ZK_SLOT_G16);
         if (rc == ZK_OK) rc = zk_msm_enqueue_sort(ctx, &nf->job, s_acc, nullptr);
-        if (rc == ZK_OK) rc = zk_groth16_witness_map_dev(ctx, r, zn, h_scratch);
+        if (rc == ZK_OK) rc = N.witness_map(ctx, zn, h_scratch);
         if (rc == ZK_OK) {
             ZK_HIP(ctx, hipEventCreateWithFlags(&nf->wm_done, hipEventDisableTiming));
             ZK_HIP(ctx, hipEventRecord(nf->wm_done, ctx->stream));
@@ -226,7 +226,7 @@
     std::unique_ptr<ZkPresort> p(new ZkPresort());
     p->pk = pk;
     p->z = z;
-    ZK_TRY(ZkG16Jobs(pk, r, z, nullptr).prepare(ctx, 0, &p->job, ZK_SLOT_G16));
+    ZK_TRY(ZkG16Jobs(pk, r, z, nullptr, true, true).prepare(ctx, 0, &p->job, ZK_SLOT_G16));
     ZK_TRY(zk_msm_enqueue_sort(ctx, &p->job, ctx->aux[0], nullptr));
     ctx->presort = p.release();
     return ZK_OK;
@@ -248,7 +248,7 @@
     (void)hipEventDestroy(e0);
     std::unique_ptr<ZkPresort> p(new ZkPresort());
     p->pk = pk; p->z = z; p->r = r; p->begun = true;
-    const ZkG16Jobs T(pk, r, z, nullptr);
+    const ZkG16Jobs T(pk, r, z, nullptr, true, true);
     ZkMsmJob* J[4] = {&p->job, &p->j1, &p->j2, &p->j3};
     int rc = T.sort_z(ctx, J, s_sort, ZK_SLOT_G16);
     if (rc == ZK_OK && !T.l_shared) rc = zk_msm_enqueue_sort(ctx, J[3], s_sort, nullptr);
diff --git a/zk-mpc_amd/csrc/groth16_prove.hip b/zk-mpc_amd/csrc/groth16_prove.hip
--- a/zk-mpc_amd/csrc/groth16_prove.hip
+++ b/zk-mpc_amd/csrc/groth16_prove.hip
@@ -35,11 +35,12 @@
 void zk_tail_chain_2(const zk_pk* pk, ZkTail* t, const zk_g2_projective& b2_sum) {
     t->b_aff = xyzz_to_affine<H2>(coeff<H2>(t->s_g2, pk->b0_g2, &b2_sum, pk->beta_g2));
 }
-void zk_tail_finish(const ZkTail& t, const zk_g1_projective& h_sum, const zk_g1_projective& l_sum, uint8_t proof[192]) {
+void zk_tail_finish(const ZkTail& t, const zk_g1_projective& h_sum, const zk_g1_projective& l_sum, uint8_t proof[192], const Affine<G1Field>* l_const) {
     X1 g_c = xyzz_add<H1>(t.s_g_a, t.r_g1_b);
     g_c = xyzz_add<H1>(g_c, xyzz_neg<H1>(t.r_s_delta));
     g_c = xyzz_add<H1>(g_c, host64_proj_from_abi<H1>((const uint64_t*)&l_sum));
     g_c = xyzz_add<H1>(g_c, host64_proj_from_abi<H1>((const uint64_t*)&h_sum));
+    if (l_const) g_c = xyzz_madd<H1>(g_c, aff_to_host64<G1Field>(*l_const));
     g1_serialize(aff_from_host64<G1Field>(xyzz_to_affine<H1>(t.g_a)), proof);
     g2_serialize(aff_from_host64<G2Field>(t.b_aff), proof + 48);
     g1_serialize(aff_from_host64<G1Field>(xyzz_to_affine<H1>(g_c)), proof + 144);
@@ -67,9 +68,9 @@
     if (pre_2.valid()) pre_2.wait();
 }
 
-void ZkProofTail::finish(const zk_g1_projective& h_sum, const zk_g1_projective& l_sum, uint8_t proof[192]) {
+void ZkProofTail::finish(const zk_g1_projective& h_sum, const zk_g1_projective& l_sum, uint8_t proof[192], const Affine<G1Field>* l_const) {
     join();
-    zk_tail_finish(t, h_sum, l_sum, proof);
+    zk_tail_finish(t, h_sum, l_sum, proof, l_const);
 }
 
 extern "C" int zk_groth16_prove_dev(zk_ctx* ctx, const zk_pk* pk, const zk_r1cs* r, const void* z, const zk_fr* r_, const zk_fr* s_,
@@ -86,7 +87,7 @@
     const auto t_tail = std::chrono::steady_clock::now();
     tail.join();
     ZK_TRY(rc_msm);
-    tail.finish(m1[0], m1[1], proof);
+    tail.finish(m1[0], m1[1], proof, ZkG16Jobs(pk, r, nullptr, nullptr).l_const);
     if (ctx->profiling) {
         auto& t = ctx->timers["host.tail"];
         t.ms += std::chrono::duration<float, std::milli>(std::chrono::steady_clock::now() - t_tail).count();
diff --git a/zk-mpc_amd/csrc/internal.hpp b/zk-mpc_amd/csrc/internal.hpp
--- a/zk-mpc_amd/csrc/internal.hpp
+++ b/zk-mpc_amd/csrc/internal.hpp
@@ -96,6 +96,7 @@
 constexpr uint32_t ZK_MSM_MAX_LEVELS = 3, ZK_MSM_MIN_LOG_NB = 6;
 extern "C" uint32_t zk_msm_mul_levels_clamp(uint32_t c, uint32_t levels);
 uint32_t zk_mul_levels_for_key(zk_ctx* ctx, size_t n);
+size_t zk_key_tables_bytes(size_t n, uint32_t M, int g1_tables);
 int zk_bases_precompute_levels(zk_ctx* ctx, zk_bases* b, uint32_t levels);
 uint32_t zk_precompute_windows(size_t n);
 int zk_bases_precompute_auto(zk_ctx* ctx, zk_bases* b);
diff --git a/zk-mpc_amd/csrc/r1cs.hip b/zk-mpc_amd/csrc/r1cs.hip
--- a/zk-mpc_amd/csrc/r1cs.hip
+++ b/zk-mpc_amd/csrc/r1cs.hip
@@ -214,6 +214,35 @@
     return zk_vec_sub_scale_launch(ctx, a, c, zinv, a, total);
 }
 
+int zk_groth16_witness_map_eval_dev(zk_ctx* ctx, const zk_r1cs* r, const void* z, void* e) {
+    if (!ctx || !r || !z || !e) return ZK_ERR_ARG;
+    const size_t D = (size_t)1 << r->log_d;
+    void* b;
+    ZK_TRY(zk_scratch(ctx, "wm_b", D * 32, &b));
+    ZK_TRY(spmv(ctx, r, 0, z, r->ni, e));
+    ZK_TRY(spmv(ctx, r, 1, z, 0, b));
+    void* v[2] = {e, b};
+    ZK_TRY(zk_ntt_launch_batch(ctx, v, 2, r->log_d, 1, 0));
+    ZK_TRY(zk_ntt_launch_batch(ctx, v, 2, r->log_d, 0, 1));
+    return zk_vec_op_launch(ctx, ZK_OP_MUL, e, b, e, D);
+}
+
+int zk_groth16_witness_map_eval_batch(zk_ctx* ctx, const zk_r1cs* r, size_t count, const void* z, void* abc) {
+    const size_t D = (size_t)1 << r->log_d, m = r->ni + r->nw, total = count * D;
+    char* a = (char*)abc;
+    char *b = a + total * 32, *tmp = b + total * 32;
+    const unsigned g = zk_grid(total, 256);
+    for (int which = 0; which < 2; which++) {
+        const auto& mt = r->m[which];
+        hipLaunchKernelGGL(k_spmv_multi, g, 256, 0, ctx->stream, mt.row_ptr, mt.col, mt.coeff, mt.all_one ? 1 : 0, z, m, r->nc,
+                           which == 0 ? r->ni : (size_t)0, r->log_d, total, (void*)(which == 0 ? a : b));
+    }
+    ZK_HIP(ctx, hipGetLastError());
+    ZK_TRY(zk_ntt_launch_strided(ctx, a, 2 * count, D, r->log_d, 1, 0, tmp));
+    ZK_TRY(zk_ntt_launch_strided(ctx, a, 2 * count, D, r->log_d, 0, 1, tmp));
+    return zk_vec_op_launch(ctx, ZK_OP_MUL, a, b, a, total);
+}
+
 extern "C" int zk_groth16_witness_map_dev(zk_ctx* ctx, const zk_r1cs* r, const void* z, void* h) {
     ZK_API_BEGIN(ctx)
     if (!ctx || !r || !z || !h) return ZK_ERR_ARG;
```

New measurement: 71.92 million constraints/s, median of 6. 2.0% higher.
